# MILVLG/mmnas

Measured on AMD Instinct MI355X. Metric: supernet fwd+bwd steps/sec (VQA arch, bs=64), higher is better.
Workload: dtype f32 (bf16x6 split-operand MFMA, fp32 accumulate); 1 GPU; Net_Search supernet WEIGHT step: sample + fwd + BCE(sum) + bwd (+ gradient all-reduce), HSIZE 256, B=64/GPU, 100x2048 regions + 14 tokens, dropout 0.1 (search_vqa.py:279-292; BASELINE configs[2]); global_batch=64, parallelism=dp1, grad_allreduce=none, rccl_ranks=1, rank_id_sum_ok=True, lstm_fallback=False, dp_rows=1, dp_buckets=3, optimizer_in_step=False, gemm_split=6, hip_force_dev_kernarg=1

## Files before the change

include/mmnas_hip.h:

```cpp
#ifndef MMNAS_HIP_H
#define MMNAS_HIP_H

#include <stddef.h>
#include <stdint.h>

#ifdef __cplusplus
extern "C" {
#endif

#define MMNAS_ABI_VERSION 1

enum {
  MMNAS_OK = 0,
  MMNAS_E_SHAPE = -1,
  MMNAS_E_ARG = -2,
  MMNAS_E_LAUNCH = -3
};

enum {
  MMNAS_F_NORM = 1,
  MMNAS_F_RESIDUAL = 2,
  MMNAS_F_MASK = 4,
  MMNAS_F_REL = 8,
  MMNAS_F_SELF = 16,
  MMNAS_F_TRAIN = 32,
  MMNAS_F_RELRAW = 64
};

int mmnas_abi_version(void);
const char* mmnas_last_error(void);

int mmnas_dropout_mask(float* out, size_t n, float p, uint64_t seed, uint32_t site, void* stream);

enum { MMNAS_GEMM_NT = 0, MMNAS_GEMM_NN = 1, MMNAS_GEMM_TN = 2 };

typedef struct mmnas_gemm_group {
  int M;
  const float* A[3];
  const float* B[3];
  float* C;
  const float* bias;
  const float* residual;
  const float* gate;
  float* colsum;
  uint64_t drop_seed;
} mmnas_gemm_group;

#define MMNAS_GEMM_MAX_GROUPS 9

typedef struct mmnas_gemm_desc {
  int layout, ngroups, nseg;
  int N, K;
  int lda, ldb, ldc, ldres, ldgate;
  int relu, split_k;
  int accumulate;
  int b_planes;
  float alpha, gate_scale;
  float drop_p;
  uint32_t drop_site;
  uint64_t drop_seed;
  mmnas_gemm_group g[MMNAS_GEMM_MAX_GROUPS];
} mmnas_gemm_desc;

int mmnas_gemm(const mmnas_gemm_desc* d, void* stream);

int mmnas_gemm_ln(const mmnas_gemm_desc* d, const float* ln_a, const float* ln_b, float* y, float eps, void* stream);
int mmnas_set_gemm_ln(int on);

int mmnas_split_planes(const float* w, void* planes, size_t n, void* stream);

int mmnas_gemm_pair(const mmnas_gemm_desc* dgrad, const mmnas_gemm_desc* wgrad, void* stream);

int mmnas_lstm_supported(int E, int H);
int mmnas_lstm_fwd(const float* x_tm, const float* Wih, const float* Whh, const float* bias, float* xp, float* Hall,
                   float* Call, float* Gall, float* out, int T, int B, int E, int H, void* stream);
int mmnas_lstm_bwd(const float* dout, const float* Whh, const float* Call, const float* Gall, float* DG, float* dc,
                   float* scratch, int T, int B, int H, void* stream);

int mmnas_lstm_seq_supported(int H, int B);
int mmnas_lstm_seq_fwd(const float* xp, const float* bhh, const float* Whh, float* Hprev, float* Cs, float* Gall,
                       float* out, int T, int B, int H, void* stream);
int mmnas_lstm_seq_bwd(const float* dout, const float* Whh, const float* Cs, const float* Gall, float* DG, int T,
                       int B, int H, void* stream);
int mmnas_lstm_seq_timed_out(void* stream);

int mmnas_gemm_reload_tuning(void);

int mmnas_layernorm_fwd(const float* x, const float* a, const float* b, float* y,
                        int M, int d, float eps, void* stream);
int mmnas_layernorm_bwd(const float* x, const float* a, const float* dy, float* dx,
                        float* da, float* db, float* ddrop, float* dcol, float* ws,
                        float drop_p, uint64_t seed, uint32_t site,
                        int M, int d, float eps, void* stream);

size_t mmnas_layernorm_bwd_ws_floats(int M, int d);

int mmnas_colsum(const float* x, float* out, int M, int N, int ldx, void* stream);

int mmnas_eltwise_fwd(int kind, const float* x, float* y, size_t n, void* stream);
int mmnas_eltwise_bwd(int kind, const float* x, const float* dy, float* dx, size_t n, void* stream);
int mmnas_drop_add(const float* x, const float* res, float* y, size_t n, float drop_p, uint64_t seed,
                   uint32_t site, void* stream);
int mmnas_glu_fwd(const float* h, float* y, int M, int C, int relu, float drop_p, uint64_t seed,
                  uint32_t site, void* stream);
int mmnas_glu_bwd(const float* h, const float* dy, float* dh, int M, int C, int relu, float drop_p,
                  uint64_t seed, uint32_t site, void* stream);

int mmnas_row_is_zero(const float* f, uint8_t* mask, long rows, int d, void* stream);
int mmnas_glimpse1_supported(int K);
size_t mmnas_glimpse1_bwd_ws_floats(long rows, int K);
int mmnas_glimpse1_fwd(const float* x, const float* w, const float* b, float* y, long rows, int K, void* stream);
int mmnas_glimpse1_bwd(const float* dy, const float* x, const float* w, float* dx, float* dw, float* db, float* ws, long rows, int K,
                       void* stream);
int mmnas_attflat_pool_fwd(const float* logits, const float* x, const uint8_t* mask, float* probs, float* pooled,
                           int B, int S, int d, int G, void* stream);
int mmnas_attflat_pool_bwd(const float* probs, const float* x, const uint8_t* mask, const float* dpooled,
                           float* dlogits, float* dx, int B, int S, int d, int G, void* stream);

int mmnas_relation_embedding(const float* bbox, const int* nobj, float* out, int B, int S, void* stream);

int mmnas_semantic_embedding(const long* ques_ix, const int* nwords, const float* emb, float* out, int B, int S,
                             int E, long V, void* stream);

int mmnas_onehot_rows(float* out, int rows, int width, const int* idx_host, void* stream);

#define MMNAS_MIXED_MAX 8
size_t mmnas_mixed_sum_ws_floats(void);
int mmnas_node_mix_fwd(const float* const* z, const float* const* ln_a, const float* const* ln_b, int n, const float* gate,
                       float* out, int M, int d, float eps, void* stream);
int mmnas_node_mix_bwd(const float* const* z, const float* const* ln_a, const float* const* ln_b, int n, const float* gate,
                       const float* dout, float* d_active, int active, float* dgate, float* ws, int M, int d, float eps,
                       void* stream);
int mmnas_mixed_sum_fwd(const float* const* outs_host, int n, const float* gate, float* out, size_t count,
                        void* stream);
int mmnas_mixed_sum_bwd(const float* const* outs_host, int n, const float* gate, const float* dout,
                        float* d_active, int active, float* dgate, float* ws, size_t count, void* stream);
int mmnas_alpha_full_step(float* prob, const float* gate_grad, float* m, float* v, float* prob_grad, int rows,
                          int width, float lr, float beta1, float beta2, float eps, int step, void* stream);

int mmnas_embedding_bwd(const long* idx, const float* dy, float* dW, long n_tok, int E, long V, void* stream);
size_t mmnas_embedding_bwd_det_ws_floats(long n_tok, int E);
int mmnas_embedding_bwd_det(const long* idx, const float* dy, float* dW, float* ws, long n_tok, int E, long V, float scale,
                            void* stream);

int mmnas_rel_bias_fwd(const float* rel, const float* Wr, const float* br, float* biasT,
                       int B, int Sq, int Sk, int R, int H, void* stream);
int mmnas_rel_bias_bwd(const float* rel, const float* Wr, const float* br, const float* dbiasT,
                       float* drel, float* dWr, float* dbr, int accumulate_drel,
                       int B, int Sq, int Sk, int R, int H, void* stream);

int mmnas_rel_fused_supported(int C, int R, int H);
int mmnas_rel_fused_fwd(const float* raw, const float* Wy, const float* by, const float* Wr,
                        const float* br, float* biasT, int B, int Sq, int Sk, int C, int R, int H,
                        void* stream);
size_t mmnas_rel_fused_bwd_ws_floats(int B, int Sq, int Sk);
int mmnas_rel_fused_bwd(const float* raw, const float* Wy, const float* by, const float* Wr,
                        const float* br, const float* dbiasT, float* dWy, float* dby, float* dWr,
                        float* dbr, float* ws, int B, int Sq, int Sk, int C, int R, int H,
                        void* stream);
int mmnas_rel_fused_fwd_ragged(const float* raw, const float* Wy, const float* by, const float* Wr, const float* br,
                               float* biasT, int B, int S, int C, int R, int H, const int* off, void* stream);
int mmnas_rel_fused_bwd_ragged(const float* raw, const float* Wy, const float* by, const float* Wr, const float* br,
                               const float* dbiasT, float* dWy, float* dby, float* dWr, float* dbr, float* ws,
                               int B, int S, int C, int R, int H, const int* off, const int* tile_off, int ntiles, void* stream);

#define MMNAS_REL_MULTI_MAX 32
typedef struct mmnas_rel_multi {
  int B, S, C, R, H, n_ops;
  const float* raw;
  const float* Wy; const float* by;
  float* dWy; float* dby;
  const float* Wr[MMNAS_REL_MULTI_MAX];
  const float* br[MMNAS_REL_MULTI_MAX];
  float* biasT[MMNAS_REL_MULTI_MAX];
  const float* dbiasT[MMNAS_REL_MULTI_MAX];
  float* dWr[MMNAS_REL_MULTI_MAX]; float* dbr[MMNAS_REL_MULTI_MAX];
  const int* off; const int* tile_off; int ntiles, reserved;
  float* ws;
} mmnas_rel_multi;
int mmnas_rel_multi_supported(int C, int R, int H);
size_t mmnas_rel_multi_bwd_ws_floats(int B, int S);
int mmnas_rel_multi_fwd(const mmnas_rel_multi* m, void* stream);
int mmnas_rel_multi_bwd(const mmnas_rel_multi* m, void* stream);
int mmnas_set_rel_hoist(int on);
int mmnas_set_guided_hoist(int on);
int mmnas_set_rel_overlap(int on);

typedef struct mmnas_mha_desc {
  int B, H, Sq, Sk, dh;
  int ldq, ldk, ldv, ldo;
  const float* Q; const float* K; const float* V;
  const uint8_t* mask;
  const float* biasT;
  float* O;
  float* lse;
  float drop_p; uint32_t drop_site; uint64_t drop_seed;
  const float* dO;
  float* dQ; float* dK; float* dV;
  float* dbiasT;
  float* delta;
  const int* q_off; const int* k_off;
} mmnas_mha_desc;

int mmnas_mha_core_fwd(const mmnas_mha_desc* d, void* stream);
int mmnas_mha_core_bwd(const mmnas_mha_desc* d, void* stream);
int mmnas_mha_core_fwd_indexed(const mmnas_mha_desc* d, const int* kv_idx, void* stream);

typedef struct mmnas_att_op {
  int B, Sq, Sk, d, di, H, dh, R;
  int flags;
  float drop_p, eps;
  uint64_t seed;
  const float* xq;
  const float* xkv;
  const uint8_t* mask;
  const float* rel;
  const float* Wq; const float* Wk; const float* Wv;
  const float* Wm;
  const float* Wr; const float* br;
  const float* ln_a; const float* ln_b;
  float* y;
  void* save;
  void* ws;
  const float* dy;
  float* dxq;
  float* dxkv;
  float* drel;
  float* dWq; float* dWk; float* dWv; float* dWm;
  float* dWr; float* dbr; float* dln_a; float* dln_b;
  int C;
  const float* Wy; const float* by;
  float* dWy; float* dby;
  const int* q_off; const int* k_off;
  int Mq, Mk;
  const int* rel_tile_off;
  int rel_ntiles, reserved2;
} mmnas_att_op;

typedef struct mmnas_plan {
  size_t save_bytes, ws_fwd_bytes, ws_bwd_bytes;
} mmnas_plan;

int mmnas_set_small_ops(int on);
int mmnas_set_small_bwd(int on);
int mmnas_set_small_ffn(int on);
int mmnas_att_op_plan(const mmnas_att_op* op, mmnas_plan* plan);
int mmnas_att_op_fwd(const mmnas_att_op* op, void* stream);
int mmnas_att_op_bwd(const mmnas_att_op* op, void* stream);

typedef struct mmnas_mlp_op {
  int M, nl;
  int dims[4];
  int flags;
  float drop_p, eps;
  uint64_t seed;
  const float* x;
  const float* W[3];
  const float* b[3];
  const float* ln_a; const float* ln_b;
  float* y;
  void* save; void* ws;
  const float* dy;
  float* dx;
  float* dW[3]; float* db[3];
  float* dln_a; float* dln_b;
} mmnas_mlp_op;

int mmnas_mlp_op_plan(const mmnas_mlp_op* op, mmnas_plan* plan);
int mmnas_mlp_op_fwd(const mmnas_mlp_op* op, void* stream);
int mmnas_mlp_op_bwd(const mmnas_mlp_op* op, void* stream);

#define MMNAS_CHAIN_MAX_OPS 128
enum { MMNAS_CHAIN_ATT = 0, MMNAS_CHAIN_MLP = 1 };
typedef struct mmnas_chain_op {
  int kind, on_y;
  mmnas_att_op att;
  mmnas_mlp_op mlp;
  int node, cand, detached, reserved;
} mmnas_chain_op;
typedef struct mmnas_chain {
  int n_ops;
  const mmnas_chain_op* ops;
  int B, Sx, Sy, d;
  const float* x_in; const float* y_in;
  const uint8_t* x_mask; const uint8_t* y_mask;
  const float* x_rel; const float* y_rel;
  void* arena;
  float* x_out; float* y_out;
  const float* dx_out; const float* dy_out;
  float* dx_in; float* dy_in;
  int use_side_stream, reserved;
  void* const* marks;
  int mixed, gate_width;
  const float* gate;
  float* dgate;
  const int* y_off;
  const int* y_tile_off;
  int Ny, y_ntiles;
} mmnas_chain;
int mmnas_chain_plan(const mmnas_chain* c, size_t* arena_bytes);
int mmnas_chain_fwd(const mmnas_chain* c, void* stream);
int mmnas_chain_bwd(const mmnas_chain* c, void* stream);
int mmnas_chain_join(void* main_stream, void* waiting_stream);
int mmnas_set_chain_overlap(int on);

typedef struct mmnas_attflat_side {
  int S, reserved;
  const float* x; const uint8_t* mask;
  const float* W1; const float* b1; const float* W2; const float* b2; const float* Wm; const float* bm;
  float* dW1; float* db1; float* dW2; float* db2; float* dWm; float* dbm;
  uint64_t seed;
  float* dx;
  const int* off;
  int M, reserved2;
} mmnas_attflat_side;
typedef struct mmnas_head {
  int B, d, MID, G, OUT, ANS, flags, reserved;
  float drop_p, eps;
  mmnas_attflat_side sx, sy;
  const float* ln_a; const float* ln_b; float* dln_a; float* dln_b;
  const float* Wp; const float* bp; float* dWp; float* dbp;
  float* logits;
  const float* dlogits;
  void* arena;
} mmnas_head;
int mmnas_head_plan(const mmnas_head* hd, size_t* arena_bytes);
int mmnas_head_fwd(const mmnas_head* hd, void* stream);
// ... 64 lines not shown
```

mmnas_amd/_lib.py:

```python
import ctypes as C
import logging
import os

import torch

_HERE = os.path.dirname(os.path.abspath(__file__))
LIB_PATH = os.environ.get('MMNAS_LIB_PATH') or os.path.join(_HERE, 'lib', 'libmmnas_hip.so')

log = logging.getLogger('mmnas_amd')


def _launch_configuration():
    name = 'HIP_FORCE_DEV_KERNARG'
    if name in os.environ:
        return os.environ[name], 'inherited'
    if torch.cuda.is_initialized():
        log.warning('mmnas_amd was imported after HIP had initialised and %s is not set: kernel arguments go through host-visible '
                    'memory, the ~300 short launches of a step run 20-40 %% slower.  Export %s=1 or import mmnas / mmnas_amd '
                    'before the first CUDA call.', name, name)
        return None, 'unset_after_hip_init'
    os.environ[name] = '1'
    return '1', 'set_by_library'


# ... 44 lines not shown


class Plan(C.Structure):
    _fields_ = [('save_bytes', C.c_size_t), ('ws_fwd_bytes', C.c_size_t), ('ws_bwd_bytes', C.c_size_t)]


class MlpOp(C.Structure):
    _fields_ = [('M', C.c_int), ('nl', C.c_int), ('dims', C.c_int * 4), ('flags', C.c_int),
                ('drop_p', C.c_float), ('eps', C.c_float), ('seed', C.c_uint64),
                ('x', _fp), ('W', _fp * 3), ('b', _fp * 3), ('ln_a', _fp), ('ln_b', _fp), ('y', _fp),
                ('save', _fp), ('ws', _fp), ('dy', _fp), ('dx', _fp), ('dW', _fp * 3), ('db', _fp * 3),
                ('dln_a', _fp), ('dln_b', _fp)]


class ChainOp(C.Structure):
    _fields_ = [('kind', C.c_int), ('on_y', C.c_int), ('att', AttOp), ('mlp', MlpOp),
                ('node', C.c_int), ('cand', C.c_int), ('detached', C.c_int), ('reserved', C.c_int)]


class Chain(C.Structure):
    _fields_ = [('n_ops', C.c_int), ('ops', C.POINTER(ChainOp)), ('B', C.c_int), ('Sx', C.c_int), ('Sy', C.c_int),
                ('d', C.c_int), ('x_in', _fp), ('y_in', _fp), ('x_mask', _fp), ('y_mask', _fp), ('x_rel', _fp),
                ('y_rel', _fp), ('arena', _fp), ('x_out', _fp), ('y_out', _fp), ('dx_out', _fp), ('dy_out', _fp),
                ('dx_in', _fp), ('dy_in', _fp), ('use_side_stream', C.c_int), ('reserved', C.c_int),
                ('marks', C.c_void_p), ('mixed', C.c_int), ('gate_width', C.c_int), ('gate', _fp), ('dgate', _fp),
                ('y_off', _fp), ('y_tile_off', _fp), ('Ny', C.c_int), ('y_ntiles', C.c_int)]


CHAIN_MAX_OPS = 128


class AttFlatSide(C.Structure):
    _fields_ = [('S', C.c_int), ('reserved', C.c_int), ('x', _fp), ('mask', _fp), ('W1', _fp), ('b1', _fp), ('W2', _fp),
                ('b2', _fp), ('Wm', _fp), ('bm', _fp), ('dW1', _fp), ('db1', _fp), ('dW2', _fp), ('db2', _fp), ('dWm', _fp),
                ('dbm', _fp), ('seed', C.c_uint64), ('dx', _fp), ('off', _fp), ('M', C.c_int), ('reserved2', C.c_int)]


class Head(C.Structure):
    _fields_ = [('B', C.c_int), ('d', C.c_int), ('MID', C.c_int), ('G', C.c_int), ('OUT', C.c_int), ('ANS', C.c_int),
                ('flags', C.c_int), ('reserved', C.c_int), ('drop_p', C.c_float), ('eps', C.c_float),
                ('sx', AttFlatSide), ('sy', AttFlatSide), ('ln_a', _fp), ('ln_b', _fp), ('dln_a', _fp), ('dln_b', _fp),
                ('Wp', _fp), ('bp', _fp), ('dWp', _fp), ('dbp', _fp), ('logits', _fp), ('dlogits', _fp), ('arena', _fp)]


REL_MULTI_MAX = 32


class RelMulti(C.Structure):
    _fields_ = [('B', C.c_int), ('S', C.c_int), ('C', C.c_int), ('R', C.c_int), ('H', C.c_int), ('n_ops', C.c_int),
                ('raw', _fp), ('Wy', _fp), ('by', _fp), ('dWy', _fp), ('dby', _fp),
                ('Wr', _fp * REL_MULTI_MAX), ('br', _fp * REL_MULTI_MAX), ('biasT', _fp * REL_MULTI_MAX),
                ('dbiasT', _fp * REL_MULTI_MAX), ('dWr', _fp * REL_MULTI_MAX), ('dbr', _fp * REL_MULTI_MAX),
                ('off', _fp), ('tile_off', _fp), ('ntiles', C.c_int), ('reserved', C.c_int), ('ws', _fp)]


class ProfStat(C.Structure):
    _fields_ = [('ms', C.c_double), ('flops', C.c_double), ('bytes', C.c_double), ('launches', C.c_long)]


K_NAMES = ['gemm', 'mha_fwd', 'mha_bwd', 'rel_fwd', 'rel_bwd', 'rowops', 'lstm', 'small_ops']


class Segment(C.Structure):
    _fields_ = [('ptr', _fp), ('offset', C.c_uint64), ('n', C.c_uint64)]


_i, _f, _u32, _u64, _sz = C.c_int, C.c_float, C.c_uint32, C.c_uint64, C.c_size_t
SYMBOLS = {
    'mmnas_abi_version': (_i, []),
    'mmnas_last_error': (C.c_char_p, []),
    'mmnas_dropout_mask': (_i, [_fp, _sz, _f, _u64, _u32, _fp]),
    'mmnas_gemm': (_i, [C.POINTER(GemmDesc), _fp]),
    'mmnas_split_planes': (_i, [_fp, _fp, _sz, _fp]),
    'mmnas_gemm_ln': (_i, [C.POINTER(GemmDesc), _fp, _fp, _fp, _f, _fp]),
    'mmnas_set_gemm_ln': (_i, [_i]),
    'mmnas_gemm_pair': (_i, [C.POINTER(GemmDesc), C.POINTER(GemmDesc), _fp]),
    'mmnas_gemm_reload_tuning': (_i, []),
    'mmnas_lstm_supported': (_i, [_i, _i]),
    'mmnas_lstm_fwd': (_i, [_fp] * 9 + [_i, _i, _i, _i, _fp]),
    'mmnas_lstm_bwd': (_i, [_fp] * 7 + [_i, _i, _i, _fp]),
    'mmnas_lstm_seq_supported': (_i, [_i, _i]),
    'mmnas_set_small_ops': (_i, [_i]),
    'mmnas_set_small_bwd': (_i, [_i]),
    'mmnas_set_small_ffn': (_i, [_i]),
    'mmnas_set_chain_overlap': (_i, [_i]),
    'mmnas_lstm_seq_fwd': (_i, [_fp] * 7 + [_i, _i, _i, _fp]),
    'mmnas_lstm_seq_bwd': (_i, [_fp] * 5 + [_i, _i, _i, _fp]),
    'mmnas_lstm_seq_timed_out': (_i, [_fp]),
    'mmnas_layernorm_fwd': (_i, [_fp, _fp, _fp, _fp, _i, _i, _f, _fp]),
    'mmnas_layernorm_bwd': (_i, [_fp, _fp, _fp, _fp, _fp, _fp, _fp, _fp, _fp, _f, _u64, _u32, _i, _i, _f, _fp]),
    'mmnas_layernorm_bwd_ws_floats': (_sz, [_i, _i]),
    'mmnas_colsum': (_i, [_fp, _fp, _i, _i, _i, _fp]),
    'mmnas_eltwise_fwd': (_i, [_i, _fp, _fp, _sz, _fp]),
    'mmnas_eltwise_bwd': (_i, [_i, _fp, _fp, _fp, _sz, _fp]),
    'mmnas_drop_add': (_i, [_fp, _fp, _fp, _sz, _f, _u64, _u32, _fp]),
    'mmnas_glu_fwd': (_i, [_fp, _fp, _i, _i, _i, _f, _u64, _u32, _fp]),
    'mmnas_glu_bwd': (_i, [_fp, _fp, _fp, _i, _i, _i, _f, _u64, _u32, _fp]),
    'mmnas_rel_bias_fwd': (_i, [_fp, _fp, _fp, _fp, _i, _i, _i, _i, _i, _fp]),
    'mmnas_rel_bias_bwd': (_i, [_fp, _fp, _fp, _fp, _fp, _fp, _fp, _i, _i, _i, _i, _i, _i, _fp]),
    'mmnas_row_is_zero': (_i, [_fp, _fp, C.c_long, _i, _fp]),
    'mmnas_glimpse1_supported': (_i, [_i]),
    'mmnas_glimpse1_bwd_ws_floats': (_sz, [C.c_long, _i]),
    'mmnas_glimpse1_fwd': (_i, [_fp, _fp, _fp, _fp, C.c_long, _i, _fp]),
    'mmnas_glimpse1_bwd': (_i, [_fp, _fp, _fp, _fp, _fp, _fp, _fp, C.c_long, _i, _fp]),
    'mmnas_attflat_pool_fwd': (_i, [_fp, _fp, _fp, _fp, _fp, _i, _i, _i, _i, _fp]),
    'mmnas_attflat_pool_bwd': (_i, [_fp, _fp, _fp, _fp, _fp, _fp, _i, _i, _i, _i, _fp]),
    'mmnas_relation_embedding': (_i, [_fp, _fp, _fp, _i, _i, _fp]),
    'mmnas_semantic_embedding': (_i, [_fp, _fp, _fp, _fp, _i, _i, _i, C.c_long, _fp]),
    'mmnas_onehot_rows': (_i, [_fp, _i, _i, C.POINTER(C.c_int), _fp]),
    'mmnas_mixed_sum_ws_floats': (_sz, []),
    'mmnas_mixed_sum_fwd': (_i, [C.POINTER(_fp), _i, _fp, _fp, _sz, _fp]),
    'mmnas_mixed_sum_bwd': (_i, [C.POINTER(_fp), _i, _fp, _fp, _fp, _i, _fp, _fp, _sz, _fp]),
    'mmnas_alpha_full_step': (_i, [_fp, _fp, _fp, _fp, _fp, _i, _i, _f, _f, _f, _f, _i, _fp]),
    'mmnas_embedding_bwd': (_i, [_fp, _fp, _fp, C.c_long, _i, C.c_long, _fp]),
    'mmnas_node_mix_fwd': (_i, [_fp, _fp, _fp, _i, _fp, _fp, _i, _i, _f, _fp]),
    'mmnas_node_mix_bwd': (_i, [_fp, _fp, _fp, _i, _fp, _fp, _fp, _i, _fp, _fp, _i, _i, _f, _fp]),
    'mmnas_embedding_bwd_det': (_i, [_fp, _fp, _fp, _fp, C.c_long, _i, C.c_long, _f, _fp]),
    'mmnas_embedding_bwd_det_ws_floats': (_sz, [C.c_long, _i]),
    'mmnas_rel_fused_supported': (_i, [_i, _i, _i]),
    'mmnas_rel_fused_fwd': (_i, [_fp, _fp, _fp, _fp, _fp, _fp, _i, _i, _i, _i, _i, _i, _fp]),
    'mmnas_rel_fused_bwd_ws_floats': (_sz, [_i, _i, _i]),
    'mmnas_rel_fused_bwd': (_i, [_fp, _fp, _fp, _fp, _fp, _fp, _fp, _fp, _fp, _fp, _fp, _i, _i, _i, _i, _i, _i, _fp]),
    'mmnas_rel_fused_fwd_ragged': (_i, [_fp, _fp, _fp, _fp, _fp, _fp, _i, _i, _i, _i, _i, _fp, _fp]),
    'mmnas_rel_fused_bwd_ragged': (_i, [_fp] * 11 + [_i, _i, _i, _i, _i, _fp, _fp, _i, _fp]),
    'mmnas_rel_multi_supported': (_i, [_i, _i, _i]),
    'mmnas_rel_multi_bwd_ws_floats': (_sz, [_i, _i]),
    'mmnas_rel_multi_fwd': (_i, [C.POINTER(RelMulti), _fp]),
    'mmnas_rel_multi_bwd': (_i, [C.POINTER(RelMulti), _fp]),
    'mmnas_set_rel_hoist': (_i, [_i]),
    'mmnas_set_guided_hoist': (_i, [_i]),
    'mmnas_set_rel_overlap': (_i, [_i]),
    'mmnas_mha_core_fwd': (_i, [C.POINTER(MhaDesc), _fp]),
    'mmnas_mha_core_bwd': (_i, [C.POINTER(MhaDesc), _fp]),
    'mmnas_mha_core_fwd_indexed': (_i, [C.POINTER(MhaDesc), _fp, _fp]),
    'mmnas_itm_pair_head': (_i, [_fp] * 11 + [C.c_long, _i, _i, _f, _fp]),
    'mmnas_rank_matrix': (_i, [_fp, _i, _i, C.c_long, _fp, _fp, _fp, _fp, _fp, _fp]),
    'mmnas_row_topk': (_i, [_fp, _i, _i, C.c_long, _i, _fp, _fp, _fp]),
    'mmnas_vgd_targets': (_i, [_fp, _fp, _fp, _i, _i, C.c_double, _i, _fp, _fp, _fp, _fp, _fp, _fp, _fp]),
    'mmnas_vgd_ground': (_i, [_fp] * 5 + [_i, _i, C.c_double] + [_fp] * 7),
    'mmnas_vqa_answer': (_i, [_fp, _i, _i, C.c_long, _fp, C.c_long, _i, _i] + [_fp] * 4 + [_i] + [_fp] * 5),
    'mmnas_vqa_accuracy': (_i, [_fp] * 4 + [_i] * 4 + [_fp, _fp, _fp]),
    'mmnas_vqa_answer_targets': (_i, [_fp, _i, _i, _i, _fp, _fp, _fp]),
    'mmnas_vgd_loss_fwd': (_i, [_fp] * 6 + [_i] * 6 + [C.c_double, C.c_double] + [_fp] * 5),
    'mmnas_itm_triplet_loss_fwd': (_i, [_fp, _fp, _fp, C.c_long, _i, _f, _i, _fp, _fp, _fp]),
    'mmnas_loss_grad_scale': (_i, [_fp, _fp, _fp, _sz, _fp]),
    'mmnas_att_op_plan': (_i, [C.POINTER(AttOp), C.POINTER(Plan)]),
    'mmnas_att_op_fwd': (_i, [C.POINTER(AttOp), _fp]),
    'mmnas_att_op_bwd': (_i, [C.POINTER(AttOp), _fp]),
    'mmnas_mlp_op_plan': (_i, [C.POINTER(MlpOp), C.POINTER(Plan)]),
    'mmnas_mlp_op_fwd': (_i, [C.POINTER(MlpOp), _fp]),
    'mmnas_mlp_op_bwd': (_i, [C.POINTER(MlpOp), _fp]),
    'mmnas_chain_plan': (_i, [C.POINTER(Chain), C.POINTER(C.c_size_t)]),
    'mmnas_chain_fwd': (_i, [C.POINTER(Chain), _fp]),
    'mmnas_chain_bwd': (_i, [C.POINTER(Chain), _fp]),
    'mmnas_chain_join': (_i, [_fp, _fp]),
    'mmnas_head_plan': (_i, [C.POINTER(Head), C.POINTER(C.c_size_t)]),
    'mmnas_head_fwd': (_i, [C.POINTER(Head), _fp]),
    'mmnas_head_bwd': (_i, [C.POINTER(Head), _fp]),
    'mmnas_bce_logits_sum_fwd': (_i, [_fp, _fp, _fp, _sz, _fp]),
    'mmnas_bce_logits_bwd': (_i, [_fp, _fp, _fp, _fp, _sz, _fp]),
    'mmnas_im2col_seq': (_i, [_fp, _fp, _i, _i, _i, _i, _fp]),
    'mmnas_pack_rows': (_i, [_fp, _fp, _fp, _i, _i, _i, _fp]),
    'mmnas_unpack_rows': (_i, [_fp, _fp, _fp, _i, _i, _i, _fp]),
    'mmnas_pad_seq': (_i, [_fp, _fp, _i, _i, _i, _i, _i, C.c_long, _fp]),
    'mmnas_col2im_seq': (_i, [_fp, _fp, _i, _i, _i, _i, _fp]),
    'mmnas_dwconv_seq_fwd': (_i, [_fp, _fp, _fp, _fp, _i, _i, _i, _i, _fp]),
    'mmnas_dwconv_seq_bwd': (_i, [_fp, _fp, _fp, _fp, _fp, _fp, _i, _i, _i, _i, _fp]),
    'mmnas_pack_segments': (_i, [_fp, _i, _fp, _f, _i, _fp]),
    'mmnas_pack_segments_host': (_i, [C.POINTER(Segment), _i, _fp, _f, _i, _fp]),
    'mmnas_adam_step': (_i, [_fp, _fp, _fp, _fp, _sz, _f, _f, _f, _f, _f, _fp, _f, _i, _fp]),
    'mmnas_sumsq': (_i, [_fp, _sz, _fp, _fp]),
    'mmnas_prof_enable': (_i, [_i]),
    'mmnas_prof_collect': (_i, [C.POINTER(ProfStat)]),
}

# ... 50 lines not shown
```

mmnas_amd/csrc/common.h:

```cpp
#pragma once
#include <hip/hip_runtime.h>
#include <hip/hip_ext.h>
#include <stdint.h>
#include <stdio.h>
#include "../../include/mmnas_hip.h"
#include "rng.h"

namespace mmnas {

typedef float f32x4 __attribute__((ext_vector_type(4)));
typedef float f32x16 __attribute__((ext_vector_type(16)));

void set_error(const char* fmt, ...);
int check_launch(const char* what);

#define MMNAS_REQUIRE(cond, code, ...) \
  do { if (!(cond)) { ::mmnas::set_error(__VA_ARGS__); return (code); } } while (0)

template <int CTRL, int ROW_MASK>
__device__ __forceinline__ float dpp_move(float old, float src) {
  return __int_as_float(__builtin_amdgcn_update_dpp(__float_as_int(old), __float_as_int(src), CTRL, ROW_MASK, 0xf, false));
}
__device__ __forceinline__ float wave_sum(float v) {
  v += dpp_move<0xB1, 0xf>(0.f, v);
  v += dpp_move<0x4E, 0xf>(0.f, v);
  v += dpp_move<0x141, 0xf>(0.f, v);
  v += dpp_move<0x140, 0xf>(0.f, v);
  v += dpp_move<0x142, 0xa>(0.f, v);
  v += dpp_move<0x143, 0xc>(0.f, v);
  return __int_as_float(__builtin_amdgcn_readlane(__float_as_int(v), 63));
}
__device__ __forceinline__ float wave_max(float v) {
  constexpr float NI = -__builtin_inff();
  v = fmaxf(v, dpp_move<0xB1, 0xf>(NI, v));
  v = fmaxf(v, dpp_move<0x4E, 0xf>(NI, v));
  v = fmaxf(v, dpp_move<0x141, 0xf>(NI, v));
  v = fmaxf(v, dpp_move<0x140, 0xf>(NI, v));
  v = fmaxf(v, dpp_move<0x142, 0xa>(NI, v));
  v = fmaxf(v, dpp_move<0x143, 0xc>(NI, v));
  return __int_as_float(__builtin_amdgcn_readlane(__float_as_int(v), 63));
}

__device__ __forceinline__ int acc_row(int r, int hh) { return (r & 3) + 8 * (r >> 2) + 4 * hh; }

__device__ __forceinline__ f32x16 mfma32(float a, float b, f32x16 c) {
  return __builtin_amdgcn_mfma_f32_32x32x2f32(a, b, c, 0, 0, 0);
}

struct ProfScope {
  ProfScope(int kind, double flops, double bytes, hipStream_t st, const char* tag = nullptr);
  ~ProfScope();
  long idx_;
  hipStream_t st_;
};

struct ProfEvents { hipEvent_t start, stop; };
ProfEvents prof_launch_events();

#define MMNAS_LAUNCH(kernel, grid, block, shmem, stream, ...)                                            \
  do {                                                                                                   \
    const ::mmnas::ProfEvents pe_ = ::mmnas::prof_launch_events();                                       \
    if (pe_.stop) hipExtLaunchKernelGGL(kernel, grid, block, shmem, stream, pe_.start, pe_.stop, 0, __VA_ARGS__); \
    else hipLaunchKernelGGL(kernel, grid, block, shmem, stream, __VA_ARGS__);                            \
  } while (0)

bool prof_enabled();

struct AuxReduce {
  const float* part;
  int nrows, d;
  float* out[3];
};
int launch_aux_reduce(const AuxReduce& a, hipStream_t st);
int gemm_pair_aux(const mmnas_gemm_desc* dgrad, const mmnas_gemm_desc* wgrad, const AuxReduce* aux, hipStream_t st);
int gemm_wgrad_aux(const mmnas_gemm_desc* wgrad, const AuxReduce* aux, hipStream_t st);
int layernorm_bwd_deferred(const float* x, const float* a, const float* dy, float* dx, float* da, float* db, float* ddrop,
                           float* dcol, float* ws, float drop_p, uint64_t seed, uint32_t site, int M, int d, float eps,
                           hipStream_t st, AuxReduce* aux);


bool gemm_ln_applies(const mmnas_gemm_desc* d);
int gemm_ln(const mmnas_gemm_desc* d, const float* ln_a, const float* ln_b, float* y, int ldy, float eps, hipStream_t st);

bool glimpse1_supported(int MID);
int glimpse1_fwd(const float* h0, const float* w0, const float* b0, float* l0, long rows0, const float* h1, const float* w1,
                 const float* b1, float* l1, long rows1, int MID, hipStream_t st);
struct NodeLnBwd {
  float* dz; float* dt;
  float* part;
  DropCfg drop;
};
int node_mix_bwd_impl(const float* const* z, const float* const* ln_a, const float* const* ln_b, int n, const float* gate,
                      const float* dout, float* d_active, int active, float* dgate, float* ws, int M, int d, float eps,
                      hipStream_t stream, bool reduce, int* nwg_out, const NodeLnBwd* lnb = nullptr);
int mixed_reduce_many(const float* const* parts, float* const* dgates, const int* nwg, const int* n, int count, hipStream_t st);
int mha_core_fwd_pair(const mmnas_mha_desc* d0, const mmnas_mha_desc* d1, hipStream_t st);
int mha_core_fwd_indexed(const mmnas_mha_desc* d, const int* kv_idx, hipStream_t st);
int transpose2d(const float* in, float* out, int R, int C, hipStream_t st);
int glimpse1_bwd_blocks(long rows, int MID);
int glimpse1_bwd(const float* dlog, const float* h, const float* w2, float gate_scale, int gated, float* dh, float* db1, float* dW2,
                 float* part, long rows, int MID, hipStream_t st, AuxReduce* aux);

int attflat_pool_fwd_packed(const float* logits, const float* x, float* probs, float* pooled, int B, int S, int d, int G, const int* off, hipStream_t st);
int attflat_pool_bwd_packed(const float* probs, const float* x, const float* dpooled, float* dlogits, float* dx, int B, int S, int d, int G,
                            const int* off, hipStream_t st);

constexpr int ADD_MANY_MAX = 24;
int add_many(const float* const* srcs, int n, float* y, size_t count, hipStream_t st);

static inline int cdiv(long a, long b) { return (int)((a + b - 1) / b); }

}
```

mmnas_amd/csrc/gemm.hip:

```cpp
#include <stddef.h>
#include <string.h>
#include <map>
#include <mutex>
#include <utility>
#include <algorithm>
#include <climits>
#include "common.h"
#include "gemm_split.h"

namespace mmnas {

struct GemmGroupK {
  int M;
  int tile0;
  const float* A[3];
  const float* B[3];
  float* C;
  const float* bias;
  const float* residual;
  const float* gate;
  float* colsum;
  uint32_t seed_lo, site_key;
};

// ... 849 lines not shown
          float val = acc[i][j][r] * p.alpha + bv;
          if (has_relu) val = fmaxf(val, 0.f);
          if (has_drop) val *= drop_mult(gdrop, (uint32_t)row * (uint32_t)h.N + (uint32_t)col);
          if (has_gate) val = gatev[r] > 0.f ? val * p.gate_scale : 0.f;
          if (has_res) val += resv[r];
          if (has_acc) val += oldv[r];
          if (cok && row < Mg) { Cp[(size_t)row * p.ldc + col] = val; cs += val; }
        }
        if (csp != nullptr) {
          cs += __shfl_xor(cs, 32, 64);
          if (hh == 0 && cok) atomicAdd(csp + col, cs);
        }
      }
    }
#ifdef MMNAS_DBG_STAMP
    asm volatile("s_waitcnt vmcnt(0)" ::: "memory");
#endif
    MMNAS_LIFE(4);
  }
}

template <int BM, int BN, bool AKC, bool BKC, bool FAST, int NS, int EPI = 0, int PF = 1, bool BDMA = false, int LEAN = 0>
__global__ void __launch_bounds__(256, NS ? (BM == 128 ? (BN == 64 ? 2 : 1) : MMNAS_OCC_NS) : (BM == 128 ? MMNAS_OCC128 : MMNAS_OCC64)) gemm_kernel(const GemmK p) {
  __shared__ __attribute__((aligned(16))) float As[GemmShape<BM, BN, NS>::A_SZ], As1[GemmShape<BM, BN, NS>::A_SZ];
  __shared__ __attribute__((aligned(16))) float Bs[GemmShape<BM, BN, NS>::B_SZ], Bs1[GemmShape<BM, BN, NS>::B_SZ];
  __shared__ int s_old;
  gemm_body<BM, BN, AKC, BKC, FAST, NS, EPI, PF, BDMA, LEAN>(p, blockIdx.x, gridDim.x, 0, As, Bs, As1, Bs1, s_old);
}

struct AuxReduceK {
  const float* part;
  float* out[3];
  int nrows, d, ncb, njobs;
};

__device__ __forceinline__ void aux_reduce_body(const AuxReduceK& a, int job, float* red ) {
  const int w = job / a.ncb, cb = job - w * a.ncb;
  float* __restrict__ out = w == 0 ? a.out[0] : (w == 1 ? a.out[1] : a.out[2]);
  if (!out) return;
  const int cl = threadIdx.x & 15, g = threadIdx.x >> 4;
  const int c = cb * 16 + cl;
  float s0 = 0.f, s1 = 0.f, s2 = 0.f, s3 = 0.f;
  if (c < a.d) {
    const float* __restrict__ p = a.part + (size_t)w * a.d + c;
    const size_t rs = (size_t)3 * a.d;
    int b = g;
    for (; b + 48 < a.nrows; b += 64) {
      s0 += p[(size_t)b * rs];
      s1 += p[(size_t)(b + 16) * rs];
      s2 += p[(size_t)(b + 32) * rs];
      s3 += p[(size_t)(b + 48) * rs];
    }
    for (; b < a.nrows; b += 16) s0 += p[(size_t)b * rs];
  }
  red[g * 17 + cl] = (s0 + s1) + (s2 + s3);
  __syncthreads();
  if (g == 0 && c < a.d) {
    float t = 0.f;
#pragma unroll
    for (int i = 0; i < 16; ++i) t += red[i * 17 + cl];
    out[c] += t;
  }
}

template <int BM, int BN, int NS, int PF = 1, int LEAN0 = 0, int LEAN1 = 0>
__global__ void __launch_bounds__(256, NS ? MMNAS_OCC_NS : MMNAS_OCC64) gemm_pair_kernel(const GemmK q0, const GemmK q1, const int nwg0,
                                                                                    const int nwg0p, const AuxReduceK aux,
                                                                                    const int naux8) {
  __shared__ __attribute__((aligned(16))) float As[GemmShape<BM, BN, NS>::A_SZ], As1[GemmShape<BM, BN, NS>::A_SZ];
  __shared__ __attribute__((aligned(16))) float Bs[GemmShape<BM, BN, NS>::B_SZ], Bs1[GemmShape<BM, BN, NS>::B_SZ];
  __shared__ int s_old;
  int bid = blockIdx.x;
  if (bid < naux8) {
    if (bid < aux.njobs) aux_reduce_body(aux, bid, As);
    return;
  }
  bid -= naux8;
  if (bid < nwg0p) {
    if (bid < nwg0) gemm_body<BM, BN, true, false, true, NS, 0, PF, false, LEAN0>(q0, bid, nwg0, 0, As, Bs, As1, Bs1, s_old);
  } else {
    gemm_body<BM, BN, false, false, true, NS, 0, PF, false, LEAN1>(q1, bid - nwg0p, (int)gridDim.x - naux8 - nwg0p, (int)sizeof(GemmK), As, Bs, As1, Bs1, s_old);
  }
}

static int env_int(const char* name, int dflt) {
  const char* e = getenv(name);
  return e && e[0] ? atoi(e) : dflt;
}

struct Tuning { int tile, generic, sk, wgs, min_units, gm, xcd, split, pair, split_slots, split_p, pf, wide_min, split_minwg, hyb_t, lean, lean_maxb; bool loaded; };
static Tuning g_tune = {0, 0, 1, 0, 4, 0, 1, 3, 1, 0, 24, 2, 200, 256, 16, 3, 8 << 20, false};
static void load_tuning() {
  g_tune.tile = env_int("MMNAS_GEMM_TILE", 0);
  g_tune.generic = getenv("MMNAS_GEMM_GENERIC") != nullptr;
  g_tune.sk = env_int("MMNAS_GEMM_SK", 1);
  g_tune.wgs = env_int("MMNAS_GEMM_WGS", 0);
  g_tune.min_units = env_int("MMNAS_GEMM_MIN_UNITS", 4);
  if (g_tune.min_units < 1) g_tune.min_units = 1;
  g_tune.gm = env_int("MMNAS_GEMM_GM", 0);
  g_tune.xcd = env_int("MMNAS_GEMM_XCD", 1);
  const int sp = env_int("MMNAS_GEMM_SPLIT", 6);
  g_tune.split = sp == 3 ? 2 : (sp == 6 ? 3 : (sp == 1 ? 1 : 0));
  g_tune.pair = env_int("MMNAS_GEMM_PAIR", 1);
  g_tune.split_slots = env_int("MMNAS_GEMM_SPLIT_SLOTS", 0);
  g_tune.split_p = env_int("MMNAS_GEMM_SPLIT_P", 24);
  if (g_tune.split_p < 1) g_tune.split_p = 1;
  g_tune.split_minwg = env_int("MMNAS_GEMM_SPLIT_MINWG", 256);
  g_tune.pf = env_int("MMNAS_GEMM_PF", 2) == 1 ? 1 : 2;
  g_tune.hyb_t = env_int("MMNAS_GEMM_HYB_T", 16);
  g_tune.wide_min = env_int("MMNAS_GEMM_WIDE_MIN", 200);
  g_tune.lean = env_int("MMNAS_GEMM_LEAN", 3);
  g_tune.lean_maxb = env_int("MMNAS_GEMM_LEAN_MAXB", 8 << 20);
  g_tune.loaded = true;
}

constexpr int MAX_WGS = 1024;
constexpr size_t WS_SLOT_FLOATS = (size_t)2 * 512 * 128 * 128;
constexpr int MAX_CNT_TILES = 1 << 16;

struct SkWorkspace { float* ws; int* cnt; };
static std::mutex g_ws_mu;
static std::map<std::pair<int, hipStream_t>, SkWorkspace> g_ws;

static int get_workspace(hipStream_t st, SkWorkspace* out) {
  int dev = 0;
  if (hipGetDevice(&dev) != hipSuccess) { set_error("gemm: hipGetDevice failed"); return MMNAS_E_LAUNCH; }
  std::lock_guard<std::mutex> lk(g_ws_mu);
  auto key = std::make_pair(dev, st);
  auto it = g_ws.find(key);
  if (it == g_ws.end()) {
    SkWorkspace w{nullptr, nullptr};
    if (hipMalloc((void**)&w.ws, WS_SLOT_FLOATS * sizeof(float)) != hipSuccess ||
        hipMalloc((void**)&w.cnt, MAX_CNT_TILES * sizeof(int)) != hipSuccess ||
        hipMemset(w.cnt, 0, MAX_CNT_TILES * sizeof(int)) != hipSuccess) {
      set_error("gemm: cannot allocate the stream-K workspace (%zu MiB)", WS_SLOT_FLOATS * sizeof(float) >> 20);
      return MMNAS_E_LAUNCH;
    }
    it = g_ws.emplace(key, w).first;
  }
  *out = it->second;
  return MMNAS_OK;
}

int sk_workspace(hipStream_t st, float** ws, size_t* ws_floats, int** cnt, int* ncnt) {
  SkWorkspace w;
  const int rc = get_workspace(st, &w);
  if (rc) return rc;
  *ws = w.ws; *ws_floats = WS_SLOT_FLOATS; *cnt = w.cnt; *ncnt = MAX_CNT_TILES;
  return MMNAS_OK;
}

template <int BM, int BN, bool FAST, int NS, int PF = 1>
static int launch(GemmK& k, int layout, int nwg, hipStream_t st) {
  dim3 grid(nwg), block(256);
  switch (layout) {
    case MMNAS_GEMM_NT: MMNAS_LAUNCH((gemm_kernel<BM, BN, true, true, FAST, NS, 0, PF>), grid, block, 0, st, k); break;
    case MMNAS_GEMM_NN: MMNAS_LAUNCH((gemm_kernel<BM, BN, true, false, FAST, NS, 0, PF>), grid, block, 0, st, k); break;
    default: MMNAS_LAUNCH((gemm_kernel<BM, BN, false, false, FAST, NS, 0, PF>), grid, block, 0, st, k); break;
  }
  return check_launch("gemm");
}

}

using namespace mmnas;

// ... 243 lines not shown
  GemmPlan pl;
  const int rc = plan_gemm(d, (hipStream_t)stream, pl);
  if (rc) return rc;
  return launch_plan(pl, (hipStream_t)stream);
}

namespace mmnas {
int gemm_pair_aux(const mmnas_gemm_desc* dgrad, const mmnas_gemm_desc* wgrad, const AuxReduce* aux, hipStream_t st) {
  GemmPlan p0, p1;
  int rc;
  if ((rc = plan_gemm(dgrad, st, p0))) return rc;
  if ((rc = plan_gemm(wgrad, st, p1))) return rc;
  const bool pair = g_tune.pair && p0.fast && p1.fast && !p0.big && !p1.big && !p0.wide && !p1.wide && p0.layout == MMNAS_GEMM_NN &&
                    p1.layout == MMNAS_GEMM_TN && p1.k.mode != MODE_STREAM;
  if (!pair) {
    if (aux && (rc = launch_aux_reduce(*aux, st))) return rc;
    if ((rc = launch_plan(p0, st))) return rc;
    return launch_plan(p1, st);
  }
  AuxReduceK ak;
  memset(&ak, 0, sizeof(ak));
  if (aux && aux->part && g_tune.pair != 3) {
    ak.part = aux->part; ak.nrows = aux->nrows; ak.d = aux->d;
    for (int i = 0; i < 3; ++i) ak.out[i] = aux->out[i];
    ak.ncb = cdiv(aux->d, 16);
    ak.njobs = 3 * ak.ncb;
  } else if (aux && (rc = launch_aux_reduce(*aux, st))) return rc;
  const int naux8 = (ak.njobs + 7) / 8 * 8;
  char tag[96] = "";
  if (prof_enabled()) snprintf(tag, sizeof(tag), "PAIR %.44s | %.40s", p0.tag, p1.tag);
  ProfScope ps(MMNAS_K_GEMM, p0.flops + p1.flops, p0.bytes + p1.bytes, st, tag);
  const int nwg0p = (p0.nwg + 7) / 8 * 8;
  dim3 grid(naux8 + nwg0p + p1.nwg), block(256);
  switch (g_tune.split) {
    case 1: MMNAS_LAUNCH((gemm_pair_kernel<64, 64, 1, 2>), grid, block, 0, st, p0.k, p1.k, p0.nwg, nwg0p, ak, naux8); break;
    case 2: MMNAS_LAUNCH((gemm_pair_kernel<64, 64, 2>), grid, block, 0, st, p0.k, p1.k, p0.nwg, nwg0p, ak, naux8); break;
    case 3:
      if (p0.lean == 3 && p1.lean) MMNAS_LAUNCH((gemm_pair_kernel<64, 64, 3, 2, 3, 1>), grid, block, 0, st, p0.k, p1.k, p0.nwg, nwg0p, ak, naux8);
      else if (p0.lean == 3) MMNAS_LAUNCH((gemm_pair_kernel<64, 64, 3, 2, 3, 0>), grid, block, 0, st, p0.k, p1.k, p0.nwg, nwg0p, ak, naux8);
      else if (p0.lean == 1 && p1.lean) MMNAS_LAUNCH((gemm_pair_kernel<64, 64, 3, 2, 1, 1>), grid, block, 0, st, p0.k, p1.k, p0.nwg, nwg0p, ak, naux8);
      else if (p0.lean == 2 && p1.lean) MMNAS_LAUNCH((gemm_pair_kernel<64, 64, 3, 2, 2, 1>), grid, block, 0, st, p0.k, p1.k, p0.nwg, nwg0p, ak, naux8);
      else if (p0.lean) MMNAS_LAUNCH((gemm_pair_kernel<64, 64, 3, 2, 2, 0>), grid, block, 0, st, p0.k, p1.k, p0.nwg, nwg0p, ak, naux8);
      else if (p1.lean) MMNAS_LAUNCH((gemm_pair_kernel<64, 64, 3, 2, 0, 1>), grid, block, 0, st, p0.k, p1.k, p0.nwg, nwg0p, ak, naux8);
      else if (g_tune.pf == 2) MMNAS_LAUNCH((gemm_pair_kernel<64, 64, 3, 2>), grid, block, 0, st, p0.k, p1.k, p0.nwg, nwg0p, ak, naux8);
      else MMNAS_LAUNCH((gemm_pair_kernel<64, 64, 3>), grid, block, 0, st, p0.k, p1.k, p0.nwg, nwg0p, ak, naux8);
      break;
    default:
      if (g_tune.pf == 2) MMNAS_LAUNCH((gemm_pair_kernel<64, 64, 0, 2>), grid, block, 0, st, p0.k, p1.k, p0.nwg, nwg0p, ak, naux8);
      else MMNAS_LAUNCH((gemm_pair_kernel<64, 64, 0>), grid, block, 0, st, p0.k, p1.k, p0.nwg, nwg0p, ak, naux8);
      break;
  }
  return check_launch("gemm_pair");
}
}

namespace mmnas {
int gemm_wgrad_aux(const mmnas_gemm_desc* wgrad, const AuxReduce* aux, hipStream_t st) {
  GemmPlan p1;
  int rc;
  if ((rc = plan_gemm(wgrad, st, p1))) return rc;
  const bool ride = aux && aux->part && g_tune.pair && g_tune.pair != 3 && g_tune.split == 3 && g_tune.pf == 2 && p1.fast && !p1.big && !p1.wide &&
                    p1.layout == MMNAS_GEMM_TN && p1.k.mode != MODE_STREAM;
  if (!ride) {
    if (aux && (rc = launch_aux_reduce(*aux, st))) return rc;
    return launch_plan(p1, st);
  }
  AuxReduceK ak;
  memset(&ak, 0, sizeof(ak));
  ak.part = aux->part; ak.nrows = aux->nrows; ak.d = aux->d;
  for (int i = 0; i < 3; ++i) ak.out[i] = aux->out[i];
  ak.ncb = cdiv(aux->d, 16);
  ak.njobs = 3 * ak.ncb;
  const int naux8 = (ak.njobs + 7) / 8 * 8;
  char tag[96] = "";
  if (prof_enabled()) snprintf(tag, sizeof(tag), "WGRAD+AUX %.60s", p1.tag);
  ProfScope ps(MMNAS_K_GEMM, p1.flops, p1.bytes, st, tag);
  dim3 grid(naux8 + p1.nwg), block(256);
  if (p1.lean) MMNAS_LAUNCH((gemm_pair_kernel<64, 64, 3, 2, 0, 1>), grid, block, 0, st, p1.k, p1.k, 0, 0, ak, naux8);
  else MMNAS_LAUNCH((gemm_pair_kernel<64, 64, 3, 2>), grid, block, 0, st, p1.k, p1.k, 0, 0, ak, naux8);
  return check_launch("gemm_wgrad_aux");
}
}

extern "C" int mmnas_gemm_pair(const mmnas_gemm_desc* dgrad, const mmnas_gemm_desc* wgrad, void* stream) {
  return gemm_pair_aux(dgrad, wgrad, nullptr, (hipStream_t)stream);
}

namespace mmnas {
__global__ void __launch_bounds__(256) split_planes_kernel(const float4* __restrict__ w, uint2* __restrict__ p0, uint2* __restrict__ p1,
                                                           uint2* __restrict__ p2, size_t n4) {
  for (size_t i = (size_t)blockIdx.x * 256 + threadIdx.x; i < n4; i += (size_t)gridDim.x * 256) {
    const float4 v = w[i];
    unsigned a0, a1, a2, b0, b1, b2;
    split_pair<3>(v.x, v.y, a0, a1, a2);
    split_pair<3>(v.z, v.w, b0, b1, b2);
    p0[i] = make_uint2(a0, b0);
    p1[i] = make_uint2(a1, b1);
    p2[i] = make_uint2(a2, b2);
  }
}
}

extern "C" int mmnas_split_planes(const float* w, void* planes, size_t n, void* stream) {
  MMNAS_REQUIRE(w && planes, MMNAS_E_ARG, "split_planes: null pointer");
  MMNAS_REQUIRE(n > 0 && n % 8 == 0 && ((uintptr_t)w & 15) == 0 && ((uintptr_t)planes & 15) == 0, MMNAS_E_SHAPE,
                "split_planes: n = %zu must be a multiple of 8 and both buffers 16-byte aligned", n);
  const size_t n4 = n / 4;
  unsigned short* pl = (unsigned short*)planes;
  const int blocks = (int)std::min<size_t>((n4 + 255) / 256, 2048);
  MMNAS_LAUNCH(split_planes_kernel, dim3(blocks), dim3(256), 0, (hipStream_t)stream, (const float4*)w, (uint2*)pl, (uint2*)(pl + n),
               (uint2*)(pl + 2 * n), n4);
  return check_launch("split_planes");
}

namespace mmnas {
static int lstm_step_plan(GemmPlan& pl, const mmnas_gemm_desc& d, hipStream_t st, const char* who, int units_per_wg) {
  int rc = plan_gemm(&d, st, pl);
  if (rc) return rc;
  MMNAS_REQUIRE(pl.fast && !pl.big && !pl.wide, MMNAS_E_SHAPE, "%s: shape outside the step kernel's range (hidden size %% 32 == 0, aligned buffers)", who);
  GemmK& k = pl.k;
  k.n_full = k.full_per = k.sk_per = 0;
  if (units_per_wg <= 0 || units_per_wg >= k.T) {
    k.mode = MODE_TILE; k.P = k.T; pl.nwg = k.ntiles;
  } else {
    SkWorkspace w;
    if ((rc = get_workspace(st, &w))) return rc;
    k.ws = w.ws; k.cnt = w.cnt;
    k.mode = MODE_STREAM; k.P = units_per_wg; k.U = k.ntiles * k.T;
    pl.nwg = (k.U + k.P - 1) / k.P;
  }
  return MMNAS_OK;
}
}

extern "C" int mmnas_lstm_supported(int E, int H) { return E > 0 && H >= 32 && H % 32 == 0 && H <= 4096; }

extern "C" int mmnas_lstm_fwd(const float* x_tm, const float* Wih, const float* Whh, const float* bias, float* xp, float* Hall,
                              float* Call, float* Gall, float* out, int T, int B, int E, int H, void* stream) {
  MMNAS_REQUIRE(x_tm && Wih && Whh && bias && xp && Hall && Call && Gall && out, MMNAS_E_ARG, "lstm_fwd: null pointer");
  MMNAS_REQUIRE(T > 0 && B > 0 && mmnas_lstm_supported(E, H), MMNAS_E_SHAPE, "lstm_fwd: T=%d B=%d E=%d H=%d", T, B, E, H);
  hipStream_t st = (hipStream_t)stream;
  mmnas_gemm_desc d;
  memset(&d, 0, sizeof(d));
  d.layout = MMNAS_GEMM_NT; d.ngroups = 1; d.nseg = 1; d.N = 4 * H; d.K = E; d.lda = E; d.ldb = E; d.ldc = 4 * H;
  d.alpha = 1.f; d.gate_scale = 1.f; d.split_k = 1;
  d.g[0].M = T * B; d.g[0].A[0] = x_tm; d.g[0].B[0] = Wih; d.g[0].C = xp; d.g[0].bias = bias;
  int rc = mmnas_gemm(&d, stream);
  if (rc) return rc;
  const size_t bh = (size_t)B * H, bg = (size_t)B * 4 * H;
  for (int t = 0; t < T; ++t) {
    memset(&d, 0, sizeof(d));
    d.layout = MMNAS_GEMM_NT; d.ngroups = 1; d.nseg = 1; d.N = 4 * H; d.K = H; d.lda = H; d.ldb = H; d.ldc = H;
    d.ldres = 4 * H; d.alpha = 1.f; d.gate_scale = 1.f; d.split_k = 1;
    d.g[0].M = B; d.g[0].A[0] = Hall + t * bh; d.g[0].B[0] = Whh; d.g[0].C = Hall + (t + 1) * bh; d.g[0].residual = xp + t * bg;
    GemmPlan pl;
    if ((rc = lstm_step_plan(pl, d, st, "lstm_fwd", env_int("MMNAS_LSTM_FWD_P", 0)))) return rc;
    pl.k.lg_cprev = Call + t * bh; pl.k.lg_cout = Call + (t + 1) * bh; pl.k.lg_gates = Gall + t * bg;
    pl.k.lg_h2 = out + (size_t)t * H; pl.k.lg_ldh2 = T * H;
    ProfScope ps(MMNAS_K_GEMM, pl.flops, pl.bytes, st, pl.tag);
    MMNAS_LAUNCH((gemm_kernel<64, 64, true, true, true, 0, 1>), dim3(pl.nwg), dim3(256), 0, st, pl.k);
  }
  return check_launch("lstm_fwd");
}

extern "C" int mmnas_lstm_bwd(const float* dout, const float* Whh, const float* Call, const float* Gall, float* DG, float* dc,
                              float* scratch, int T, int B, int H, void* stream) {
// ... 32 lines not shown
```

mmnas_amd/csrc/ops.hip:

```cpp
#include <string.h>
#include <functional>
#include <vector>
#include "common.h"

namespace mmnas {

static inline size_t al(size_t n) { return (n + 255) & ~(size_t)255; }

struct Carver {
  char* base; size_t off;
  explicit Carver(void* p) : base((char*)p), off(0) {}
  float* take(size_t nfloats) { float* r = (float*)(base + off); off += al(nfloats * sizeof(float)); return r; }
};

static void gemm_init(mmnas_gemm_desc& g, int layout, int N, int K, int lda, int ldb, int ldc) {
  memset(&g, 0, sizeof(g));
  g.layout = layout; g.ngroups = 1; g.nseg = 1; g.N = N; g.K = K; g.lda = lda; g.ldb = ldb; g.ldc = ldc;
  g.alpha = 1.f; g.gate_scale = 1.f; g.split_k = 1;
}

struct AttLayout {
  size_t Mq, Mk;
  float *Q, *K, *V, *att, *stats, *z, *biasT;
  float *dz, *dt, *datt, *dQ, *dK, *dV, *delta, *dbiasT, *lnws, *relws;
// ... 121 lines not shown
      rc = op->q_off ? mmnas_rel_fused_fwd_ragged(op->rel, op->Wy, op->by, op->Wr, op->br, L.biasT, op->B, op->Sq, op->C, op->R,
                                                  op->H, op->q_off, stream)
                     : mmnas_rel_fused_fwd(op->rel, op->Wy, op->by, op->Wr, op->br, L.biasT, op->B, op->Sq, op->Sk, op->C, op->R,
                                           op->H, stream);
    } else {
      rc = mmnas_rel_bias_fwd(op->rel, op->Wr, op->br, L.biasT, op->B, op->Sq, op->Sk, op->R, op->H, stream);
    }
    if (rc) return rc;
  }
  if (desc_only) { att_core_desc(op, L, desc_only); return MMNAS_OK; }
  mmnas_mha_desc m;
  att_core_desc(op, L, &m);
  return mmnas_mha_core_fwd(&m, stream);
}

static void att_merge_group(const mmnas_att_op* op, const AttLayout& L, mmnas_gemm_group* g) {
  const bool norm = op->flags & MMNAS_F_NORM;
  memset(g, 0, sizeof(*g));
  g->M = (int)L.Mq; g->A[0] = L.att; g->B[0] = op->Wm; g->C = norm ? L.z : op->y;
  if (op->flags & MMNAS_F_RESIDUAL) g->residual = op->xq;
  g->drop_seed = op->seed;
}

static int att_fwd_args(const mmnas_att_op* op) {
  int rc = att_check(op, "att_op_fwd");
  if (rc) return rc;
  MMNAS_REQUIRE(op->xq && op->xkv && op->Wq && op->Wk && op->Wv && op->Wm && op->y && op->save, MMNAS_E_ARG,
                "att_op_fwd: null pointer");
  const int fl = op->flags;
  if (fl & MMNAS_F_NORM) MMNAS_REQUIRE(op->ln_a && op->ln_b, MMNAS_E_ARG, "att_op_fwd: NORM without ln parameters");
  if (fl & MMNAS_F_REL) MMNAS_REQUIRE(op->rel && op->Wr && op->br, MMNAS_E_ARG, "att_op_fwd: REL without rel/Wr/br");
  if (fl & MMNAS_F_MASK) MMNAS_REQUIRE(op->mask, MMNAS_E_ARG, "att_op_fwd: MASK without mask");
  return MMNAS_OK;
}
}

static int mmnas::att_fwd_impl(const mmnas_att_op* op, void* stream, bool defer_ln, bool* ln_done, bool rel_ready, bool kv_ready) {
  *ln_done = true;
  int rc = att_fwd_args(op);
  if (rc) return rc;
  const int fl = op->flags;
  const bool norm = fl & MMNAS_F_NORM;
  const bool drop = (fl & MMNAS_F_TRAIN) && op->drop_p > 0.f;
  AttLayout L = att_layout(op);
  const int d = op->d, di = op->di;
  if (sa_small_applies(op)) return sa_small_fwd(op, L.Q, L.K, L.V, L.att, L.stats, L.z, (hipStream_t)stream);

  mmnas_gemm_desc g;
  gemm_init(g, MMNAS_GEMM_NT, di, d, d, d, di);
  g.ngroups = kv_ready ? 1 : 3;
  att_qkv_groups(op, L, g.g);
  if ((rc = mmnas_gemm(&g, stream))) return rc;
  if ((rc = att_core_fwd(op, L, stream, nullptr, rel_ready))) return rc;
  gemm_init(g, MMNAS_GEMM_NT, d, di, di, di, d);
  att_merge_group(op, L, &g.g[0]);
  if (fl & MMNAS_F_RESIDUAL) g.ldres = d;
  if (drop) { g.drop_p = op->drop_p; g.drop_site = 1; g.drop_seed = op->seed; }
  if (norm && !defer_ln && gemm_ln_applies(&g)) return gemm_ln(&g, op->ln_a, op->ln_b, op->y, d, op->eps, (hipStream_t)stream);
  if ((rc = mmnas_gemm(&g, stream))) return rc;

  if (norm && defer_ln) { *ln_done = false; return MMNAS_OK; }
  if (norm) return mmnas_layernorm_fwd(L.z, op->ln_a, op->ln_b, op->y, (int)L.Mq, d, op->eps, stream);
  return MMNAS_OK;
}

namespace mmnas {
struct SideQueue {
  std::vector<std::function<int(hipStream_t)>> work;
  bool rel_only = false;
  int flush(hipStream_t main, hipStream_t side, hipEvent_t ev) {
    if (work.empty()) return MMNAS_OK;
    hipStream_t s = side;
    if (hipEventRecord(ev, main) != hipSuccess || hipStreamWaitEvent(side, ev, 0) != hipSuccess)
      s = main;
    for (auto& f : work) {
      const int rc = f(s);
      if (rc) return rc;
    }
    work.clear();
    return MMNAS_OK;
  }
};

static int att_bwd_impl(const mmnas_att_op* op, hipStream_t stream, SideQueue* sq, bool acc_kv = false, bool rel_defer = false, bool kv_defer = false,
                        const AuxReduce* ln_pre = nullptr) {
  const bool side = sq != nullptr && !sq->rel_only;
  const bool side_rel = sq != nullptr;
  int rc = att_check(op, "att_op_bwd");
  if (rc) return rc;
  MMNAS_REQUIRE(op->xq && op->xkv && op->Wq && op->Wk && op->Wv && op->Wm && op->save && op->ws && op->dy &&
                    op->dxq && op->dWq && op->dWk && op->dWv && op->dWm,
                MMNAS_E_ARG, "att_op_bwd: null pointer");
  const int fl = op->flags;
  const bool norm = fl & MMNAS_F_NORM, rel = fl & MMNAS_F_REL, self = fl & MMNAS_F_SELF;
  const bool drop = (fl & MMNAS_F_TRAIN) && op->drop_p > 0.f;
  if (!self) MMNAS_REQUIRE(op->dxkv, MMNAS_E_ARG, "att_op_bwd: dxkv required unless SELF");
  if (norm) MMNAS_REQUIRE(op->ln_a && op->dln_a && op->dln_b, MMNAS_E_ARG, "att_op_bwd: NORM gradients missing");
  if (rel) MMNAS_REQUIRE(op->rel && op->Wr && op->br && op->dWr && op->dbr, MMNAS_E_ARG, "att_op_bwd: REL gradients missing");
  AttLayout L = att_layout(op);
  const int d = op->d, di = op->di, Mq = (int)L.Mq, Mk = (int)L.Mk;

  if (!ln_pre && !sq && self && !rel && sa_small_bwd_applies(op)) {
    float* const dt_out = drop ? L.dt : (norm ? L.dz : nullptr);
    if ((rc = sa_small_bwd(op, L.Q, L.K, L.V, L.stats, L.z, dt_out, L.dQ, L.dK, L.dV, norm ? L.lnws : nullptr, stream))) return rc;
    mmnas_gemm_desc w4;
    gemm_init(w4, MMNAS_GEMM_TN, d, Mq, d, d, d);
    w4.ngroups = 4;
    w4.g[0].M = d; w4.g[0].A[0] = dt_out ? dt_out : op->dy; w4.g[0].B[0] = L.att; w4.g[0].C = op->dWm;
    w4.g[1].M = d; w4.g[1].A[0] = L.dQ; w4.g[1].B[0] = op->xq; w4.g[1].C = op->dWq;
    w4.g[2].M = d; w4.g[2].A[0] = L.dK; w4.g[2].B[0] = op->xq; w4.g[2].C = op->dWk;
    w4.g[3].M = d; w4.g[3].A[0] = L.dV; w4.g[3].B[0] = op->xq; w4.g[3].C = op->dWv;
    w4.accumulate = 1;
    AuxReduce red;
    red.part = norm ? L.lnws : nullptr; red.nrows = op->B; red.d = d;
    red.out[0] = op->dln_a; red.out[1] = op->dln_b; red.out[2] = nullptr;
    return gemm_wgrad_aux(&w4, &red, stream);
  }

  const float* dz = op->dy;
  const float* dt = op->dy;
  AuxReduce lnred;
  lnred.part = nullptr;
  if (norm && ln_pre) {
    lnred = *ln_pre;
    dz = L.dz; dt = drop ? L.dt : L.dz;
  } else if (norm) {
    if ((rc = layernorm_bwd_deferred(L.z, op->ln_a, op->dy, L.dz, op->dln_a, op->dln_b, drop ? L.dt : nullptr, nullptr,
                                     L.lnws, drop ? op->drop_p : 0.f, op->seed, 1, Mq, d, op->eps, (hipStream_t)stream, &lnred)))
      return rc;
    dz = L.dz; dt = drop ? L.dt : L.dz;
  } else if (drop) {
    if ((rc = mmnas_drop_add(op->dy, nullptr, L.dt, (size_t)Mq * d, op->drop_p, op->seed, 1, stream))) return rc;
    dt = L.dt;
  }

  mmnas_gemm_desc g, w, wm, w2;
  gemm_init(g, MMNAS_GEMM_NN, di, d, d, di, di);
  g.g[0].M = Mq; g.g[0].A[0] = dt; g.g[0].B[0] = op->Wm; g.g[0].C = L.datt;
  gemm_init(wm, MMNAS_GEMM_TN, di, Mq, d, di, di);
  wm.g[0].M = d; wm.g[0].A[0] = dt; wm.g[0].B[0] = L.att; wm.g[0].C = op->dWm;
  wm.accumulate = 1;
  if (side) { if ((rc = mmnas_gemm(&g, stream))) return rc; }
  else if ((rc = gemm_pair_aux(&g, &wm, &lnred, (hipStream_t)stream))) return rc;

  mmnas_mha_desc m;
  memset(&m, 0, sizeof(m));
  m.B = op->B; m.H = op->H; m.Sq = op->Sq; m.Sk = op->Sk; m.dh = op->dh;
  m.ldq = m.ldk = m.ldv = m.ldo = di;
  m.Q = L.Q; m.K = L.K; m.V = L.V; m.mask = (fl & MMNAS_F_MASK) ? op->mask : nullptr; m.biasT = L.biasT;
  m.O = L.att; m.lse = L.stats;
  m.drop_p = drop ? op->drop_p : 0.f; m.drop_site = 0; m.drop_seed = op->seed;
  m.dO = L.datt; m.dQ = L.dQ; m.dK = L.dK; m.dV = L.dV; m.dbiasT = L.dbiasT; m.delta = L.delta;
  m.q_off = op->q_off; m.k_off = op->k_off;
  if ((rc = mmnas_mha_core_bwd(&m, stream))) return rc;

  if (self) {
    gemm_init(w, MMNAS_GEMM_TN, d, Mq, di, d, d);
    w.ngroups = 3;
    w.g[0].M = di; w.g[0].A[0] = L.dQ; w.g[0].B[0] = op->xq;  w.g[0].C = op->dWq;
    w.g[1].M = di; w.g[1].A[0] = L.dK; w.g[1].B[0] = op->xkv; w.g[1].C = op->dWk;
    w.g[2].M = di; w.g[2].A[0] = L.dV; w.g[2].B[0] = op->xkv; w.g[2].C = op->dWv;
    w.accumulate = 1;
    gemm_init(g, MMNAS_GEMM_NN, d, di, di, d, d);
    g.nseg = 3;
    g.g[0].M = Mq; g.g[0].C = op->dxq;
    g.g[0].A[0] = L.dQ; g.g[0].B[0] = op->Wq;
    g.g[0].A[1] = L.dK; g.g[0].B[1] = op->Wk;
    g.g[0].A[2] = L.dV; g.g[0].B[2] = op->Wv;
    if (fl & MMNAS_F_RESIDUAL) { g.g[0].residual = dz; g.ldres = d; }
    if (side) {
      if ((rc = mmnas_gemm(&g, stream))) return rc;
    } else if ((rc = mmnas_gemm_pair(&g, &w, stream))) return rc;
  } else {
    gemm_init(w, MMNAS_GEMM_TN, d, Mq, di, d, d);
    w.g[0].M = di; w.g[0].A[0] = L.dQ; w.g[0].B[0] = op->xq; w.g[0].C = op->dWq;
    w.accumulate = 1;
    gemm_init(g, MMNAS_GEMM_NN, d, di, di, d, d);
    g.g[0].M = Mq; g.g[0].C = op->dxq; g.g[0].A[0] = L.dQ; g.g[0].B[0] = op->Wq;
    if (fl & MMNAS_F_RESIDUAL) { g.g[0].residual = dz; g.ldres = d; }
    if (side) {
      if ((rc = mmnas_gemm(&g, stream))) return rc;
    } else if ((rc = mmnas_gemm_pair(&g, &w, stream))) return rc;
    if (kv_defer) goto params;
    gemm_init(w2, MMNAS_GEMM_TN, d, Mk, di, d, d);
    w2.ngroups = 2;
    w2.g[0].M = di; w2.g[0].A[0] = L.dK; w2.g[0].B[0] = op->xkv; w2.g[0].C = op->dWk;
    w2.g[1].M = di; w2.g[1].A[0] = L.dV; w2.g[1].B[0] = op->xkv; w2.g[1].C = op->dWv;
    w2.accumulate = 1;
    gemm_init(g, MMNAS_GEMM_NN, d, di, di, d, d);
    g.nseg = 2;
    g.g[0].M = Mk; g.g[0].C = op->dxkv;
    g.g[0].A[0] = L.dK; g.g[0].B[0] = op->Wk;
    g.g[0].A[1] = L.dV; g.g[0].B[1] = op->Wv;
    if (acc_kv) g.accumulate = 1;
    if (side) {
      if ((rc = mmnas_gemm(&g, stream))) return rc;
    } else if ((rc = mmnas_gemm_pair(&g, &w2, stream))) return rc;
  }

params:
  if (side) {
    sq->work.push_back([lnred](hipStream_t s) { return launch_aux_reduce(lnred, s); });
    sq->work.push_back([wm](hipStream_t s) { return mmnas_gemm(&wm, s); });
    sq->work.push_back([w](hipStream_t s) { return mmnas_gemm(&w, s); });
    if (!self) sq->work.push_back([w2](hipStream_t s) { return mmnas_gemm(&w2, s); });
  }
  if (rel && rel_defer) return MMNAS_OK;
  if (rel && (fl & MMNAS_F_RELRAW)) {
    MMNAS_REQUIRE(op->Wy && op->by && op->dWy && op->dby, MMNAS_E_ARG, "att_op_bwd: RELRAW gradients missing");
    const mmnas_att_op o = *op;
    float* const dbiasT = L.dbiasT;
    float* const relws = L.relws;
    auto relb = [o, dbiasT, relws](hipStream_t s) {
      if (o.q_off)
        return mmnas_rel_fused_bwd_ragged(o.rel, o.Wy, o.by, o.Wr, o.br, dbiasT, o.dWy, o.dby, o.dWr, o.dbr, relws, o.B, o.Sq,
                                          o.C, o.R, o.H, o.q_off, o.rel_tile_off, o.rel_ntiles, s);
      return mmnas_rel_fused_bwd(o.rel, o.Wy, o.by, o.Wr, o.br, dbiasT, o.dWy, o.dby, o.dWr, o.dbr, relws, o.B, o.Sq, o.Sk,
                                 o.C, o.R, o.H, s);
    };
    if (side_rel) { sq->work.push_back(relb); return MMNAS_OK; }
    return relb(stream);
  }
  if (rel)
    return mmnas_rel_bias_bwd(op->rel, op->Wr, op->br, L.dbiasT, op->drel, op->dWr, op->dbr, 0, op->B, op->Sq,
                              op->Sk, op->R, op->H, stream);
  return MMNAS_OK;
}
}

extern "C" int mmnas_att_op_bwd(const mmnas_att_op* op, void* stream) {
  return att_bwd_impl(op, (hipStream_t)stream, nullptr);
}

namespace mmnas {

struct MlpLayout {
  float* h[3];
  float* z;
  float *dz, *dt, *dp[3], *lnws;
  size_t save_bytes, ws_bwd_bytes;
};

static MlpLayout mlp_layout(const mmnas_mlp_op* op) {
  MlpLayout L;
  const bool norm = op->flags & MMNAS_F_NORM;
  const bool drop = (op->flags & MMNAS_F_TRAIN) && op->drop_p > 0.f;
  const size_t M = (size_t)op->M;
  Carver s(op->save);
  L.h[0] = nullptr;
  for (int i = 1; i < 3; ++i) L.h[i] = (i < op->nl) ? s.take(M * op->dims[i]) : nullptr;
  L.z = norm ? s.take(M * op->dims[0]) : nullptr;
  L.save_bytes = s.off;
  size_t maxh = 4;
  for (int i = 1; i < op->nl; ++i) if ((size_t)op->dims[i] > maxh) maxh = op->dims[i];
  Carver w(op->ws);
  L.dz = norm ? w.take(M * op->dims[0]) : nullptr;
  L.dt = drop ? w.take(M * op->dims[0]) : nullptr;
  L.dp[0] = w.take(M * maxh);
  L.dp[1] = op->nl > 2 ? w.take(M * maxh) : nullptr;
  L.dp[2] = nullptr;
  L.lnws = norm ? w.take(mmnas_layernorm_bwd_ws_floats(op->M, op->dims[0])) : nullptr;
  L.ws_bwd_bytes = w.off;
  return L;
}

static int mlp_check(const mmnas_mlp_op* op, const char* who) {
  MMNAS_REQUIRE(op, MMNAS_E_ARG, "%s: null descriptor", who);
  MMNAS_REQUIRE(op->nl >= 1 && op->nl <= 3 && op->M > 0, MMNAS_E_SHAPE, "%s: nl=%d M=%d", who, op->nl, op->M);
  MMNAS_REQUIRE(op->dims[0] == op->dims[op->nl], MMNAS_E_SHAPE, "%s: in/out width differ (%d vs %d)", who,
                op->dims[0], op->dims[op->nl]);
  for (int i = 0; i <= op->nl; ++i)
    MMNAS_REQUIRE(op->dims[i] > 0 && op->dims[i] % 4 == 0, MMNAS_E_SHAPE, "%s: dims[%d]=%d", who, i, op->dims[i]);
  return MMNAS_OK;
}

}

extern "C" int mmnas_mlp_op_plan(const mmnas_mlp_op* op, mmnas_plan* plan) {
  int rc = mlp_check(op, "mlp_op_plan");
  if (rc) return rc;
  MMNAS_REQUIRE(plan, MMNAS_E_ARG, "mlp_op_plan: null plan");
  mmnas_mlp_op tmp = *op;
  tmp.save = nullptr; tmp.ws = nullptr;
  MlpLayout L = mlp_layout(&tmp);
  plan->save_bytes = L.save_bytes ? L.save_bytes : 256;
  plan->ws_fwd_bytes = 256;
  plan->ws_bwd_bytes = L.ws_bwd_bytes;
  return MMNAS_OK;
}

namespace mmnas {
static int mlp_fwd_impl(const mmnas_mlp_op* op, void* stream, bool defer_ln, bool* ln_done);
}
extern "C" int mmnas_mlp_op_fwd(const mmnas_mlp_op* op, void* stream) {
  bool done;
  return mmnas::mlp_fwd_impl(op, stream, false, &done);
}
static int mmnas::mlp_fwd_impl(const mmnas_mlp_op* op, void* stream, bool defer_ln, bool* ln_done) {
  *ln_done = true;
  int rc = mlp_check(op, "mlp_op_fwd");
  if (rc) return rc;
  MMNAS_REQUIRE(op->x && op->y && op->save, MMNAS_E_ARG, "mlp_op_fwd: null pointer");
  const int fl = op->flags;
  const bool norm = fl & MMNAS_F_NORM;
  const bool drop = (fl & MMNAS_F_TRAIN) && op->drop_p > 0.f;
  if (norm) MMNAS_REQUIRE(op->ln_a && op->ln_b, MMNAS_E_ARG, "mlp_op_fwd: NORM without ln parameters");
  MlpLayout L = mlp_layout(op);
  const int d = op->dims[0];
  if (!(norm && defer_ln) && ffn_small_applies(op)) return ffn_small_fwd(op, L.h[1], L.z, (hipStream_t)stream);
  const float* in = op->x;
  mmnas_gemm_desc g;
  for (int i = 0; i < op->nl; ++i) {
    MMNAS_REQUIRE(op->W[i], MMNAS_E_ARG, "mlp_op_fwd: W[%d] null", i);
    const bool last = i == op->nl - 1;
    gemm_init(g, MMNAS_GEMM_NT, op->dims[i + 1], op->dims[i], op->dims[i], op->dims[i], op->dims[i + 1]);
    g.g[0].M = op->M; g.g[0].A[0] = in; g.g[0].B[0] = op->W[i]; g.g[0].bias = op->b[i];
    if (drop) { g.drop_p = op->drop_p; g.drop_seed = op->seed; g.drop_site = last ? 1u : (i == 0 ? 0u : 2u); }
    if (last) {
      g.g[0].C = norm ? L.z : op->y;
      if (fl & MMNAS_F_RESIDUAL) { g.g[0].residual = op->x; g.ldres = d; }
    } else {
      g.relu = 1;
      g.g[0].C = L.h[i + 1];
    }
    if (last && norm && !defer_ln && gemm_ln_applies(&g)) return gemm_ln(&g, op->ln_a, op->ln_b, op->y, d, op->eps, (hipStream_t)stream);
    if ((rc = mmnas_gemm(&g, stream))) return rc;
    in = L.h[i + 1];
  }
  if (norm && defer_ln) { *ln_done = false; return MMNAS_OK; }
  if (norm) return mmnas_layernorm_fwd(L.z, op->ln_a, op->ln_b, op->y, op->M, d, op->eps, stream);
  return MMNAS_OK;
}

namespace mmnas {
static int mlp_bwd_impl(const mmnas_mlp_op* op, hipStream_t stream, SideQueue* sq, const AuxReduce* ln_pre = nullptr) {
  const bool side = sq != nullptr && !sq->rel_only;
  int rc = mlp_check(op, "mlp_op_bwd");
  if (rc) return rc;
  MMNAS_REQUIRE(op->x && op->save && op->ws && op->dy && op->dx, MMNAS_E_ARG, "mlp_op_bwd: null pointer");
  const int fl = op->flags;
  const bool norm = fl & MMNAS_F_NORM;
  const bool drop = (fl & MMNAS_F_TRAIN) && op->drop_p > 0.f;
  MlpLayout L = mlp_layout(op);
  const int d = op->dims[0], M = op->M, nl = op->nl;
  for (int i = 0; i < nl; ++i)
    MMNAS_REQUIRE(op->W[i] && op->dW[i], MMNAS_E_ARG, "mlp_op_bwd: W/dW[%d] null", i);

  const float* dz = op->dy;
  const float* dt = op->dy;
  bool last_bias_done = false;
  AuxReduce lnred;
  lnred.part = nullptr;
  if (norm) {
    MMNAS_REQUIRE(op->ln_a && op->dln_a && op->dln_b, MMNAS_E_ARG, "mlp_op_bwd: NORM gradients missing");
    float* dcol = (drop && op->db[nl - 1]) ? op->db[nl - 1] : nullptr;
    if (ln_pre) lnred = *ln_pre;
    else if ((rc = layernorm_bwd_deferred(L.z, op->ln_a, op->dy, L.dz, op->dln_a, op->dln_b, drop ? L.dt : nullptr, dcol,
                                          L.lnws, drop ? op->drop_p : 0.f, op->seed, 1, M, d, op->eps, (hipStream_t)stream, &lnred)))
      return rc;
    dz = L.dz; dt = drop ? L.dt : L.dz;
    last_bias_done = dcol != nullptr;
  } else if (drop) {
    if ((rc = mmnas_drop_add(op->dy, nullptr, L.dt, (size_t)M * d, op->drop_p, op->seed, 1, stream))) return rc;
    dt = L.dt;
  }

  const float gate_scale = drop ? 1.0f / (1.0f - op->drop_p) : 1.0f;
  const float* dpre = dt;
  mmnas_gemm_desc g;
  mmnas_gemm_desc wd[3];
  const bool last_colsum = op->db[nl - 1] && !last_bias_done;
  if (last_colsum && !side)
    if ((rc = mmnas_colsum(dpre, op->db[nl - 1], M, op->dims[nl], op->dims[nl], stream))) return rc;
  for (int i = nl - 1; i >= 0; --i) {
    const float* hin = i == 0 ? op->x : L.h[i];
    const int nout = op->dims[i + 1], nin = op->dims[i];
    mmnas_gemm_desc& w = wd[i];
    gemm_init(w, MMNAS_GEMM_TN, nin, M, nout, nin, nin);
    w.g[0].M = nout; w.g[0].A[0] = dpre; w.g[0].B[0] = hin; w.g[0].C = op->dW[i];
    w.accumulate = 1;
    gemm_init(g, MMNAS_GEMM_NN, nin, nout, nout, nin, nin);
    g.g[0].M = M; g.g[0].A[0] = dpre; g.g[0].B[0] = op->W[i];
    if (i == 0) {
      g.g[0].C = op->dx;
      if (fl & MMNAS_F_RESIDUAL) { g.g[0].residual = dz; g.ldres = d; }
    } else {
      float* out = L.dp[(nl - 1 - i) % 3];
      g.g[0].C = out;
      g.g[0].gate = L.h[i]; g.ldgate = nin; g.gate_scale = gate_scale;
      g.g[0].colsum = op->db[i - 1];
    }
    if (side) {
      if ((rc = mmnas_gemm(&g, stream))) return rc;
    } else if ((rc = gemm_pair_aux(&g, &w, i == nl - 1 ? &lnred : nullptr, (hipStream_t)stream))) return rc;
    if (i > 0) dpre = g.g[0].C;
  }
  if (side) {
    sq->work.push_back([lnred](hipStream_t s) { return launch_aux_reduce(lnred, s); });
    if (last_colsum) {
      float* const db = op->db[nl - 1];
      const int n = op->dims[nl];
      sq->work.push_back([dt, db, M, n](hipStream_t s) { return mmnas_colsum(dt, db, M, n, n, s); });
    }
    for (int i = nl - 1; i >= 0; --i) {
      const mmnas_gemm_desc w = wd[i];
      sq->work.push_back([w](hipStream_t s) { return mmnas_gemm(&w, s); });
    }
  }
  return MMNAS_OK;
}
}

extern "C" int mmnas_mlp_op_bwd(const mmnas_mlp_op* op, void* stream) {
  return mlp_bwd_impl(op, (hipStream_t)stream, nullptr);
}

#include <map>
#include <mutex>
#include <utility>
namespace mmnas {

struct ChainLayout {
  size_t y[MMNAS_CHAIN_MAX_OPS], save[MMNAS_CHAIN_MAX_OPS], ws[MMNAS_CHAIN_MAX_OPS], dx[MMNAS_CHAIN_MAX_OPS],
      tmp[MMNAS_CHAIN_MAX_OPS];
  size_t dpre, encdy, relws, total;
  int last_x, last_y, first_x, first_y, n_guided;
  size_t nout[MMNAS_CHAIN_MAX_OPS], ndact[MMNAS_CHAIN_MAX_OPS], mixws;
};

static int chain_check(const mmnas_chain* c, const char* who) {
  MMNAS_REQUIRE(c && c->ops, MMNAS_E_ARG, "%s: null chain", who);
  MMNAS_REQUIRE(c->n_ops >= 1 && c->n_ops <= MMNAS_CHAIN_MAX_OPS, MMNAS_E_SHAPE, "%s: %d operators (1..%d)", who, c->n_ops, MMNAS_CHAIN_MAX_OPS);
  MMNAS_REQUIRE(c->B > 0 && c->Sx > 0 && c->Sy > 0 && c->d > 0, MMNAS_E_SHAPE, "%s: B=%d Sx=%d Sy=%d d=%d", who, c->B, c->Sx, c->Sy, c->d);
  if (c->y_off) MMNAS_REQUIRE(c->Ny > 0 && c->Ny <= c->B * c->Sy && c->Sy <= 128 && !c->use_side_stream, MMNAS_E_ARG,
                              "%s: ragged decoder stream: Ny=%d of B*Sy=%d rows, Sy=%d <= 128, single stream", who, c->Ny, c->B * c->Sy, c->Sy);
  bool seen_y = false;
  for (int i = 0; i < c->n_ops; ++i) {
    const mmnas_chain_op& o = c->ops[i];
    MMNAS_REQUIRE(o.kind == MMNAS_CHAIN_ATT || o.kind == MMNAS_CHAIN_MLP, MMNAS_E_ARG, "%s: operator %d: kind %d", who, i, o.kind);
    if (o.on_y) seen_y = true;
    else MMNAS_REQUIRE(!seen_y, MMNAS_E_ARG, "%s: encoder operators must precede the decoder's (operator %d)", who, i);
    if (o.kind == MMNAS_CHAIN_ATT && !(o.att.flags & MMNAS_F_SELF))
      MMNAS_REQUIRE(o.on_y, MMNAS_E_ARG, "%s: operator %d: guided attention needs the decoder stream", who, i);
  }
  if (c->mixed) {
    MMNAS_REQUIRE(c->gate && c->gate_width >= 1 && c->gate_width <= MMNAS_MIXED_MAX, MMNAS_E_ARG, "%s: mixed chain without a gate block (width %d)", who, c->gate_width);
    MMNAS_REQUIRE(!c->use_side_stream, MMNAS_E_ARG, "%s: mixed chains run on one stream", who);
    MMNAS_REQUIRE(c->d <= 1024, MMNAS_E_SHAPE, "%s: mixed chains need d <= 1024", who);
    int node = -1, live = 0, count = 0;
    for (int i = 0; i < c->n_ops; ++i) {
      const mmnas_chain_op& o = c->ops[i];
      if (o.node != node) {
        MMNAS_REQUIRE(o.node == node + 1, MMNAS_E_ARG, "%s: operator %d: node %d after node %d", who, i, o.node, node);
        MMNAS_REQUIRE(node < 0 || live == 1, MMNAS_E_ARG, "%s: node %d has %d differentiated candidates (exactly one)", who, node, live);
        node = o.node; live = 0; count = 0;
      } else {
        MMNAS_REQUIRE(o.on_y == c->ops[i - 1].on_y, MMNAS_E_ARG, "%s: node %d mixes the two streams", who, node);
      }
      MMNAS_REQUIRE(o.cand >= 0 && o.cand < c->gate_width, MMNAS_E_ARG, "%s: operator %d: candidate %d outside the gate row", who, i, o.cand);
      MMNAS_REQUIRE(++count <= MMNAS_MIXED_MAX, MMNAS_E_SHAPE, "%s: node %d has more than %d candidates", who, node, MMNAS_MIXED_MAX);
      live += o.detached ? 0 : 1;
    }
    MMNAS_REQUIRE(live == 1, MMNAS_E_ARG, "%s: node %d has %d differentiated candidates (exactly one)", who, node, live);
  }
  return MMNAS_OK;
}

static inline size_t chain_rows_y(const mmnas_chain* c) { return c->y_off ? (size_t)c->Ny : (size_t)c->B * c->Sy; }

static void chain_op_setup(const mmnas_chain* c, int i, mmnas_att_op& a, mmnas_mlp_op& m) {
  const mmnas_chain_op& o = c->ops[i];
  const int S = o.on_y ? c->Sy : c->Sx;
  if (o.kind == MMNAS_CHAIN_ATT) {
    a = o.att;
    a.B = c->B; a.d = c->d; a.Sq = S;
    const bool self = a.flags & MMNAS_F_SELF;
    a.Sk = self ? S : c->Sx;
// ... 411 lines not shown
      }
      gemm_init(g, MMNAS_GEMM_NT, c->d, f.di, f.di, f.di, c->d);
      g.ngroups = ng;
      for (int j = 0; j < ng; ++j) att_merge_group(&ga[j], gl[j], &g.g[j]);
      if (f.flags & MMNAS_F_RESIDUAL) g.ldres = c->d;
      if (drop) { g.drop_p = f.drop_p; g.drop_site = 1; g.drop_seed = f.seed; }
      if ((rc = mmnas_gemm(&g, st))) return rc;
    }
    for (int i = i0; i < i1; ++i) {
      const mmnas_chain_op& o = c->ops[i];
      mmnas_att_op a; mmnas_mlp_op m;
      chain_op_setup(c, i, a, m);
      bool ln_done = true;
      bool staged = false;
      for (int j = 0; j < ng; ++j) staged |= gidx[j] == i;
      if (staged) {
        ln_done = !(a.flags & MMNAS_F_NORM);
        if (a.flags & MMNAS_F_NORM) eps = a.eps;
        chain_cand_view(c, L, i, ln_done, &z[i - i0], &la[i - i0], &lb[i - i0]);
        continue;
      }
      if (o.kind == MMNAS_CHAIN_ATT) {
        a.xq = cur;
        a.xkv = (a.flags & MMNAS_F_SELF) ? cur : cur_x;
        a.y = (float*)(base + L.y[i]); a.save = base + L.save[i]; a.ws = base + L.ws[i];
        if ((rc = att_fwd_impl(&a, st, true, &ln_done, RG.hoisted[i]))) return rc;
        if (a.flags & MMNAS_F_NORM) eps = a.eps;
      } else {
        m.x = cur; m.y = (float*)(base + L.y[i]); m.save = base + L.save[i]; m.ws = base + L.ws[i];
        if ((rc = mlp_fwd_impl(&m, st, true, &ln_done))) return rc;
        if (m.flags & MMNAS_F_NORM) eps = m.eps;
      }
      chain_cand_view(c, L, i, ln_done, &z[i - i0], &la[i - i0], &lb[i - i0]);
    }
    const float* zs[MMNAS_MIXED_MAX] = {nullptr}; const float* as[MMNAS_MIXED_MAX] = {nullptr}; const float* bs[MMNAS_MIXED_MAX] = {nullptr};
    int width = 0;
    for (int i = i0; i < i1; ++i) {
      const int k = c->ops[i].cand;
      zs[k] = z[i - i0]; as[k] = la[i - i0]; bs[k] = lb[i - i0];
      if (k + 1 > width) width = k + 1;
    }
    float* out = i0 == L.last_x ? c->x_out : (i0 == L.last_y ? c->y_out : (float*)(base + L.nout[i0]));
    const int M = oy ? (int)chain_rows_y(c) : c->B * c->Sx;
    if ((rc = mmnas_node_mix_fwd(zs, as, bs, width, c->gate + (size_t)c->ops[i0].node * c->gate_width, out, M, c->d, eps, st))) return rc;
    if (oy) cur_y = out; else cur_x = out;
    i0 = i1;
  }
  if (L.last_x < 0 && hipMemcpyAsync(c->x_out, c->x_in, nx, hipMemcpyDeviceToDevice, st) != hipSuccess) return MMNAS_E_LAUNCH;
  if (L.last_y < 0 && hipMemcpyAsync(c->y_out, c->y_in, ny, hipMemcpyDeviceToDevice, st) != hipSuccess) return MMNAS_E_LAUNCH;
  return MMNAS_OK;
}

static int chain_bwd_mixed(const mmnas_chain* c, hipStream_t st, const ChainLayout& L) {
  MMNAS_REQUIRE(c->dgate, MMNAS_E_ARG, "chain_bwd: mixed chain without a gate-gradient block");
  char* base = (char*)c->arena;
  const size_t ex = (size_t)c->B * c->Sx * c->d, ey = chain_rows_y(c) * c->d;
  float* dpre = (float*)(base + L.dpre);
  int rc;
  GuidedSet GS;
  chain_guided_set(c, true, true, GS);
  int Gm = -1;
  for (int i = 0; i < c->n_ops && Gm < 0; ++i)
    if (GS.hoisted[i]) Gm = i;
  const float* enc_grad = nullptr;
  if (L.n_guided > GS.n && hipMemsetAsync(dpre, 0, ex * sizeof(float), st) != hipSuccess) return MMNAS_E_LAUNCH;
  int starts[MMNAS_CHAIN_MAX_OPS + 1], nn = 0;
  for (int i = 0; i < c->n_ops; ++i)
    if (i == 0 || c->ops[i].node != c->ops[i - 1].node) starts[nn++] = i;
  starts[nn] = c->n_ops;
  auto node_out = [&](int i0) -> const float* { return i0 == L.last_x ? c->x_out : (i0 == L.last_y ? c->y_out : (const float*)(base + L.nout[i0])); };
  auto input_of = [&](int k) -> const float* {
    const bool oy = c->ops[starts[k]].on_y;
    for (int j = k - 1; j >= 0; --j)
      if ((bool)c->ops[starts[j]].on_y == oy) return node_out(starts[j]);
    return oy ? c->y_in : c->x_in;
  };
  const float* x_final = L.last_x >= 0 ? c->x_out : c->x_in;
  const float* cur_dy = c->dy_out;
  const float* red_part[MMNAS_CHAIN_MAX_OPS]; float* red_out[MMNAS_CHAIN_MAX_OPS]; int red_nwg[MMNAS_CHAIN_MAX_OPS], red_n[MMNAS_CHAIN_MAX_OPS];
  int n_red = 0;
  RelGroups RG;
  chain_rel_groups(c, L, true, RG);
  SideCtx* rel_bwd_side = nullptr;
  for (int k = nn - 1; k >= 0; --k) {
    const int i0 = starts[k], i1 = starts[k + 1];
    const bool oy = c->ops[i0].on_y;
    if (!oy && i0 == L.last_x) {
      MMNAS_REQUIRE(c->dx_out || L.n_guided, MMNAS_E_ARG, "chain_bwd: no gradient reaches the encoder (dx_out NULL, no guided operator)");
      if (enc_grad) cur_dy = enc_grad;
      else if (c->dx_out && L.n_guided) {
        float* g0 = (float*)(base + L.encdy);
        if ((rc = mmnas_drop_add(c->dx_out, dpre, g0, ex, 0.f, 0, 0, st))) return rc;
        cur_dy = g0;
      } else cur_dy = c->dx_out ? c->dx_out : dpre;
    }
    const float* zs[MMNAS_MIXED_MAX] = {nullptr}; const float* as[MMNAS_MIXED_MAX] = {nullptr}; const float* bs[MMNAS_MIXED_MAX] = {nullptr};
    int width = 0, act = -1, act_op = -1;
    float eps = 1e-6f;
    for (int i = i0; i < i1; ++i) {
      const int kc = c->ops[i].cand;
      chain_cand_view(c, L, i, chain_ln_done_in_op(c, i), &zs[kc], &as[kc], &bs[kc]);
      if (kc + 1 > width) width = kc + 1;
      if (!c->ops[i].detached) { act = kc; act_op = i; }
      const mmnas_chain_op& o = c->ops[i];
      if (o.kind == MMNAS_CHAIN_ATT) { if (o.att.flags & MMNAS_F_NORM) eps = o.att.eps; }
      else if (o.mlp.flags & MMNAS_F_NORM) eps = o.mlp.eps;
    }
    const float* nin = input_of(k);
    float* dact = (float*)(base + L.ndact[i0]);
    const int M = oy ? (int)chain_rows_y(c) : c->B * c->Sx;
    const size_t grow = (size_t)c->ops[i0].node * c->gate_width;
    const mmnas_chain_op& o = c->ops[act_op];
    mmnas_att_op a; mmnas_mlp_op m;
    chain_op_setup(c, act_op, a, m);
    float* dx = i0 == L.first_x ? c->dx_in : (i0 == L.first_y ? c->dy_in : (float*)(base + L.dx[act_op]));
    NodeLnBwd lnb;
    lnb.dz = nullptr;
    AuxReduce lnpre;
    lnpre.part = nullptr;
    if (o.kind == MMNAS_CHAIN_ATT) {
      const bool self = a.flags & MMNAS_F_SELF;
      a.xq = nin;
      a.xkv = self ? nin : x_final;
      a.save = base + L.save[act_op]; a.ws = base + L.ws[act_op];
      a.dy = dact; a.dxq = dx;
      a.dxkv = self ? nullptr : dpre;
      a.drel = nullptr;
      if (node_lnb_on() && (a.flags & MMNAS_F_NORM) && c->d <= 256 && !(self && !(a.flags & MMNAS_F_REL) && sa_small_bwd_applies(&a))) {
        const AttLayout AL = att_layout(&a);
        const bool drop = (a.flags & MMNAS_F_TRAIN) && a.drop_p > 0.f;
        lnb.dz = AL.dz; lnb.dt = drop ? AL.dt : nullptr; lnb.part = AL.lnws;
        lnb.drop = make_drop(drop ? a.drop_p : 0.f, a.seed, 1);
        lnpre.part = AL.lnws; lnpre.d = c->d;
        lnpre.out[0] = a.dln_a; lnpre.out[1] = a.dln_b; lnpre.out[2] = nullptr;
      }
    } else {
      m.x = nin; m.save = base + L.save[act_op]; m.ws = base + L.ws[act_op];
      m.dy = dact; m.dx = dx;
      if (node_lnb_on() && (m.flags & MMNAS_F_NORM) && c->d <= 256) {
        const MlpLayout ML = mlp_layout(&m);
        const bool drop = (m.flags & MMNAS_F_TRAIN) && m.drop_p > 0.f;
        lnb.dz = ML.dz; lnb.dt = drop ? ML.dt : nullptr; lnb.part = ML.lnws;
        lnb.drop = make_drop(drop ? m.drop_p : 0.f, m.seed, 1);
        lnpre.part = ML.lnws; lnpre.d = c->d;
        lnpre.out[0] = m.dln_a; lnpre.out[1] = m.dln_b; lnpre.out[2] = (drop && m.db[m.nl - 1]) ? m.db[m.nl - 1] : nullptr;
      }
    }
    {
      float* wsk = (float*)(base + L.mixws) + (size_t)k * mmnas_mixed_sum_ws_floats();
      int nwg = 0;
      if ((rc = node_mix_bwd_impl(zs, as, bs, width, c->gate + grow, cur_dy, dact, act, c->dgate + grow, wsk, M, c->d, eps, st, false, &nwg,
                                  lnb.dz ? &lnb : nullptr)))
        return rc;
      if (nwg > 0) { red_part[n_red] = wsk; red_out[n_red] = c->dgate + grow; red_nwg[n_red] = nwg; red_n[n_red] = width; ++n_red; }
      lnpre.nrows = nwg;
    }
    if (o.kind == MMNAS_CHAIN_ATT) {
      const bool self = a.flags & MMNAS_F_SELF;
      if ((rc = att_bwd_impl(&a, st, nullptr, !self, RG.hoisted[act_op], GS.hoisted[act_op], lnb.dz ? &lnpre : nullptr))) return rc;
      if (GS.n && act_op == Gm) {
        float* g0 = (float*)(base + L.encdy);
        if ((rc = chain_guided_kv_bwd(c, L, GS, x_final, c->dx_out, GS.n < L.n_guided ? dpre : nullptr, g0, st))) return rc;
        enc_grad = g0;
      }
    } else {
      if ((rc = mlp_bwd_impl(&m, st, nullptr, lnb.dz ? &lnpre : nullptr))) return rc;
    }
    cur_dy = dx;
    hipStream_t mark_stream = st;
    if (i0 == L.first_y && !RG.groups[1].empty()) {
      SideCtx* rsc = (rel_overlap_on() && L.last_x >= 0) ? side_ctx(st, true) : nullptr;
      if (rsc) {
        if ((rc = ev_fork(st, rsc->side, rsc->ovl[2]))) return rc;
        if ((rc = chain_rel_bwd(RG, 1, rsc->side))) return rc;
        rel_bwd_side = rsc;
        mark_stream = rsc->side;
      } else if ((rc = chain_rel_bwd(RG, 1, st))) return rc;
    }
    if (i0 == L.first_x && !RG.groups[0].empty()) {
      if (rel_bwd_side) { if ((rc = ev_fork(rel_bwd_side->side, st, rel_bwd_side->ovl[3]))) return rc; rel_bwd_side = nullptr; }
      if ((rc = chain_rel_bwd(RG, 0, st))) return rc;
    }
    if (c->marks && c->marks[act_op] && hipEventRecord((hipEvent_t)c->marks[act_op], mark_stream) != hipSuccess) {
      set_error("chain_bwd: cannot record the mark event of operator %d", act_op);
      return MMNAS_E_LAUNCH;
    }
  }
  if (rel_bwd_side && (rc = ev_fork(rel_bwd_side->side, st, rel_bwd_side->ovl[3]))) return rc;
  if (n_red && (rc = mixed_reduce_many(red_part, red_out, red_nwg, red_n, n_red, st))) return rc;
  if (L.first_y < 0 && hipMemcpyAsync(c->dy_in, c->dy_out, ey * sizeof(float), hipMemcpyDeviceToDevice, st) != hipSuccess) return MMNAS_E_LAUNCH;
  if (L.first_x < 0) {
    const float* g0 = c->dx_out;
    if (enc_grad) g0 = enc_grad;
    else if (c->dx_out && L.n_guided) {
      if ((rc = mmnas_drop_add(c->dx_out, dpre, c->dx_in, ex, 0.f, 0, 0, st))) return rc;
      g0 = nullptr;
    } else if (!c->dx_out) g0 = dpre;
    if (g0 && hipMemcpyAsync(c->dx_in, g0, ex * sizeof(float), hipMemcpyDeviceToDevice, st) != hipSuccess) return MMNAS_E_LAUNCH;
  }
  return MMNAS_OK;
}
}

extern "C" int mmnas_chain_fwd(const mmnas_chain* c, void* stream) {
  int rc = chain_check(c, "chain_fwd");
  if (rc) return rc;
  MMNAS_REQUIRE(c->x_in && c->y_in && c->x_out && c->y_out && c->arena, MMNAS_E_ARG, "chain_fwd: null pointer");
  hipStream_t st = (hipStream_t)stream;
  ChainLayout L;
  if ((rc = chain_layout(c, L))) return rc;
  if (c->mixed) return chain_fwd_mixed(c, st, L);
  char* base = (char*)c->arena;
  const float* cur_x = c->x_in;
  const float* cur_y = c->y_in;
  const size_t nx = (size_t)c->B * c->Sx * c->d * sizeof(float), ny = chain_rows_y(c) * c->d * sizeof(float);
  RelGroups RG;
  chain_rel_groups(c, L, false, RG);
  const int G = first_guided(c);
  const bool ovl = chain_overlap_on() && !c->use_side_stream && L.last_x >= 0 && L.first_y >= 0 && G > L.first_y;
  int rel_join_at = -1;
  SideCtx* rsc = nullptr;
  if (!ovl && rel_overlap_on() && !RG.groups[1].empty() && L.last_x >= 0 && (rsc = side_ctx(st, true)) != nullptr) {
    for (int i = L.first_y; i < c->n_ops && rel_join_at < 0; ++i)
      if (RG.hoisted[i] && c->ops[i].on_y) rel_join_at = i;
  }
  if (rel_join_at >= 0) {
    if ((rc = ev_fork(st, rsc->side, rsc->ovl[0]))) return rc;
    if ((rc = chain_rel_fwd(RG, rsc->side, 1))) return rc;
    if ((rc = chain_rel_fwd(RG, st, 0))) return rc;
  } else if ((rc = chain_rel_fwd(RG, st))) return rc;
  GuidedSet GS;
  chain_guided_set(c, false, !ovl, GS);
  auto run = [&](int i, hipStream_t s) -> int {
    const mmnas_chain_op& o = c->ops[i];
    mmnas_att_op a; mmnas_mlp_op m;
    chain_op_setup(c, i, a, m);
    const float* cur = o.on_y ? cur_y : cur_x;
    float* out = i == L.last_x ? c->x_out : (i == L.last_y ? c->y_out : (float*)(base + L.y[i]));
    int r;
    if (o.kind == MMNAS_CHAIN_ATT) {
      a.xq = cur;
      a.xkv = (a.flags & MMNAS_F_SELF) ? cur : cur_x;
      a.y = out; a.save = base + L.save[i]; a.ws = base + L.ws[i];
      bool done;
      if ((r = att_fwd_impl(&a, s, false, &done, RG.hoisted[i], GS.hoisted[i]))) return r;
    } else {
      m.x = cur; m.y = out; m.save = base + L.save[i]; m.ws = base + L.ws[i];
      if ((r = mmnas_mlp_op_fwd(&m, s))) return r;
    }
    if (o.on_y) cur_y = out; else cur_x = out;
    return MMNAS_OK;
  };
  if (!ovl) {
    for (int i = 0; i < c->n_ops; ++i) {
      if (GS.n && i == G && (rc = chain_guided_kv_fwd(c, L, GS, cur_x, st))) return rc;
      if (i == rel_join_at && (rc = ev_fork(rsc->side, st, rsc->ovl[1]))) return rc;
      if ((rc = run(i, st))) return rc;
    }
  } else {
    SideCtx* sc = side_ctx(st, true);
    MMNAS_REQUIRE(sc, MMNAS_E_LAUNCH, "chain_fwd: cannot create the encoder stream");
    if ((rc = ev_fork(st, sc->enc, sc->ovl[0]))) return rc;
    int ie = L.first_x, id = L.first_y;
    while (ie <= L.last_x || id < G) {
      if (ie <= L.last_x && (rc = run(ie++, sc->enc))) return rc;
      if (id < G && (rc = run(id++, st))) return rc;
    }
    if ((rc = ev_fork(sc->enc, st, sc->ovl[1]))) return rc;
    for (int i = G; i < c->n_ops; ++i)
      if ((rc = run(i, st))) return rc;
  }
  if (L.last_x < 0 && hipMemcpyAsync(c->x_out, c->x_in, nx, hipMemcpyDeviceToDevice, st) != hipSuccess) return MMNAS_E_LAUNCH;
  if (L.last_y < 0 && hipMemcpyAsync(c->y_out, c->y_in, ny, hipMemcpyDeviceToDevice, st) != hipSuccess) return MMNAS_E_LAUNCH;
  return MMNAS_OK;
}

extern "C" int mmnas_chain_bwd(const mmnas_chain* c, void* stream) {
  int rc = chain_check(c, "chain_bwd");
  if (rc) return rc;
  MMNAS_REQUIRE(c->x_in && c->y_in && c->x_out && c->y_out && c->arena && c->dy_out && c->dx_in && c->dy_in, MMNAS_E_ARG,
                "chain_bwd: null pointer");
  hipStream_t st = (hipStream_t)stream;
  ChainLayout L;
  if ((rc = chain_layout(c, L))) return rc;
  if (c->mixed) return chain_bwd_mixed(c, st, L);
  SideCtx* sc = c->use_side_stream ? side_ctx(st, true) : nullptr;
  MMNAS_REQUIRE(!c->use_side_stream || sc, MMNAS_E_LAUNCH, "chain_bwd: cannot create the side stream");
  hipStream_t side = sc ? sc->side : nullptr;
  if (sc) sc->used = true;
  SideQueue q;
  q.rel_only = c->use_side_stream == 2;
  SideQueue* sq = sc ? &q : nullptr;
  static const bool per_op = getenv("MMNAS_SIDE_FLUSH") && !strcmp(getenv("MMNAS_SIDE_FLUSH"), "op");
  char* base = (char*)c->arena;
  const size_t ex = (size_t)c->B * c->Sx * c->d, ey = chain_rows_y(c) * c->d;
  float* dpre = (float*)(base + L.dpre);
  auto input_of = [&](int i) -> const float* {
    const bool oy = c->ops[i].on_y;
    for (int j = i - 1; j >= 0; --j)
      if ((bool)c->ops[j].on_y == oy) return j == L.last_x ? c->x_out : (j == L.last_y ? c->y_out : (const float*)(base + L.y[j]));
    return oy ? c->y_in : c->x_in;
  };
  const float* x_final = L.last_x >= 0 ? c->x_out : c->x_in;
  const int G = first_guided(c);
  const bool ovl = chain_overlap_on() && !c->use_side_stream && L.last_x >= 0 && L.first_y >= 0 && G > L.first_y;
  RelGroups RG;
  if (!ovl) chain_rel_groups(c, L, true, RG);
  GuidedSet GS;
  chain_guided_set(c, true, !ovl, GS);
  const float* enc_grad = nullptr;
  SideCtx* rel_bwd_side = nullptr;
  if (L.n_guided > GS.n && hipMemsetAsync(dpre, 0, ex * sizeof(float), st) != hipSuccess) return MMNAS_E_LAUNCH;
  auto run = [&](int i, hipStream_t s, const float* dyi, const float** dxo) -> int {
    const mmnas_chain_op& o = c->ops[i];
    mmnas_att_op a; mmnas_mlp_op m;
    chain_op_setup(c, i, a, m);
    float* dx = i == L.first_x ? c->dx_in : (i == L.first_y ? c->dy_in : (float*)(base + L.dx[i]));
    int r;
    if (o.kind == MMNAS_CHAIN_ATT) {
      const bool self = a.flags & MMNAS_F_SELF;
      a.xq = input_of(i);
      a.xkv = self ? a.xq : x_final;
      a.save = base + L.save[i]; a.ws = base + L.ws[i];
      a.dy = dyi; a.dxq = dx;
      a.dxkv = self ? nullptr : dpre;
      a.drel = nullptr;
      if ((r = att_bwd_impl(&a, s, sq, !self, RG.hoisted[i], GS.hoisted[i]))) return r;
      if (GS.n && i == G) {
        float* g0 = (float*)(base + L.encdy);
        if ((r = chain_guided_kv_bwd(c, L, GS, x_final, c->dx_out, GS.n < L.n_guided ? dpre : nullptr, g0, s))) return r;
        enc_grad = g0;
      }
    } else {
      m.x = input_of(i); m.save = base + L.save[i]; m.ws = base + L.ws[i];
      m.dy = dyi; m.dx = dx;
      if ((r = mlp_bwd_impl(&m, s, sq))) return r;
    }
    *dxo = dx;
    hipStream_t mark_stream = s;
    if (i == L.first_y && !RG.groups[1].empty()) {
      SideCtx* rsc = (rel_overlap_on() && L.last_x >= 0 && !sq) ? side_ctx(st, true) : nullptr;
      if (rsc) {
        if ((r = ev_fork(s, rsc->side, rsc->ovl[2]))) return r;
        if ((r = chain_rel_bwd(RG, 1, rsc->side))) return r;
        rel_bwd_side = rsc;
        mark_stream = rsc->side;
      } else if ((r = chain_rel_bwd(RG, 1, s))) return r;
    }
    if (i == L.first_x && !RG.groups[0].empty()) {
      if (rel_bwd_side) { if ((r = ev_fork(rel_bwd_side->side, s, rel_bwd_side->ovl[3]))) return r; rel_bwd_side = nullptr; }
      if ((r = chain_rel_bwd(RG, 0, s))) return r;
    }
    if (!ovl && c->marks && c->marks[i] && hipEventRecord((hipEvent_t)c->marks[i], mark_stream) != hipSuccess) {
      set_error("chain_bwd: cannot record the mark event of operator %d", i);
      return MMNAS_E_LAUNCH;
    }
    return MMNAS_OK;
  };
  auto encoder_dy = [&](hipStream_t s, const float** out) -> int {
    MMNAS_REQUIRE(c->dx_out || L.n_guided, MMNAS_E_ARG, "chain_bwd: no gradient reaches the encoder (dx_out NULL, no guided operator)");
    if (enc_grad) { *out = enc_grad; return MMNAS_OK; }
    if (c->dx_out && L.n_guided) {
      float* g0 = (float*)(base + L.encdy);
      const int r = mmnas_drop_add(c->dx_out, dpre, g0, ex, 0.f, 0, 0, s);
      if (r) return r;
      *out = g0;
    } else *out = c->dx_out ? c->dx_out : dpre;
    return MMNAS_OK;
  };
  const float* cur_dy = c->dy_out;
  if (!ovl) {
    for (int i = c->n_ops - 1; i >= 0; --i) {
      if (sq && i == L.last_x && (rc = q.flush(st, side, sc->ev[0]))) return rc;
      if (!c->ops[i].on_y && i == L.last_x && (rc = encoder_dy(st, &cur_dy))) return rc;
      if ((rc = run(i, st, cur_dy, &cur_dy))) return rc;
      if (sq && per_op && (rc = q.flush(st, side, sc->ev[i + 1]))) return rc;
    }
    if (sq && (rc = q.flush(st, side, sc->ev[1]))) return rc;
  } else {
    SideCtx* oc = side_ctx(st, true);
    MMNAS_REQUIRE(oc, MMNAS_E_LAUNCH, "chain_bwd: cannot create the encoder stream");
    for (int i = c->n_ops - 1; i >= G; --i)
      if ((rc = run(i, st, cur_dy, &cur_dy))) return rc;
    if ((rc = ev_fork(st, oc->enc, oc->ovl[2]))) return rc;
    const float* enc_dy = nullptr;
    if ((rc = encoder_dy(oc->enc, &enc_dy))) return rc;
    int ie = L.last_x, id = G - 1;
    while (ie >= L.first_x || id >= L.first_y) {
      if (ie >= L.first_x && (rc = run(ie--, oc->enc, enc_dy, &enc_dy))) return rc;
      if (id >= L.first_y && (rc = run(id--, st, cur_dy, &cur_dy))) return rc;
    }
    if ((rc = ev_fork(oc->enc, st, oc->ovl[3]))) return rc;
    if (c->marks)
      for (int i = 0; i < c->n_ops; ++i)
        if (c->marks[i] && hipEventRecord((hipEvent_t)c->marks[i], st) != hipSuccess) {
          set_error("chain_bwd: cannot record the mark event of operator %d", i);
          return MMNAS_E_LAUNCH;
        }
  }
  if (rel_bwd_side && (rc = ev_fork(rel_bwd_side->side, st, rel_bwd_side->ovl[3]))) return rc;
  if (L.first_y < 0 && hipMemcpyAsync(c->dy_in, c->dy_out, ey * sizeof(float), hipMemcpyDeviceToDevice, st) != hipSuccess) return MMNAS_E_LAUNCH;
  if (L.first_x < 0) {
    const float* g0 = c->dx_out;
    if (enc_grad) g0 = enc_grad;
    else if (c->dx_out && L.n_guided) {
      if ((rc = mmnas_drop_add(c->dx_out, dpre, c->dx_in, ex, 0.f, 0, 0, stream))) return rc;
      g0 = nullptr;
    } else if (!c->dx_out) g0 = dpre;
    if (g0 && hipMemcpyAsync(c->dx_in, g0, ex * sizeof(float), hipMemcpyDeviceToDevice, st) != hipSuccess) return MMNAS_E_LAUNCH;
  }
  return MMNAS_OK;
}

extern "C" int mmnas_chain_join(void* main_stream, void* waiting_stream) {
  SideCtx* sc = side_ctx((hipStream_t)main_stream, false);
  if (!sc || !sc->used) return MMNAS_OK;
  hipEvent_t e = sc->ev[MMNAS_CHAIN_MAX_OPS];
  if (hipEventRecord(e, sc->side) != hipSuccess || hipStreamWaitEvent((hipStream_t)waiting_stream, e, 0) != hipSuccess) {
    set_error("chain_join: event record / wait failed");
    return MMNAS_E_LAUNCH;
  }
  return MMNAS_OK;
}

namespace mmnas {

struct HeadSideLayout { float *h, *logit, *probs, *pooled, *dpooled, *dlog, *dh, *dxpool, *g1part; };
static inline int head_rows(const mmnas_head* hd, const mmnas_attflat_side& sd) { return sd.off ? sd.M : hd->B * sd.S; }
struct HeadLayout {
  HeadSideLayout s[2];
  float *xo, *sum, *xy, *dxy, *dsum, *lnws, *g1proj, *dlogT;
  size_t total;
};

static HeadLayout head_layout(const mmnas_head* hd) {
  HeadLayout L;
  Carver c(hd->arena);
  const size_t B = hd->B;
  for (int k = 0; k < 2; ++k) {
    const mmnas_attflat_side& sd = k ? hd->sy : hd->sx;
    const size_t M = sd.off ? (size_t)sd.M : B * sd.S;
    HeadSideLayout& s = L.s[k];
    s.h = c.take(M * hd->MID); s.logit = c.take(M * hd->G); s.probs = c.take(M * hd->G); s.pooled = c.take(B * hd->G * hd->d);
    s.dpooled = c.take(B * hd->G * hd->d); s.dlog = c.take(M * hd->G); s.dh = c.take(M * hd->MID); s.dxpool = c.take(M * hd->d);
    s.g1part = (hd->G == 1 && glimpse1_supported(hd->MID)) ? c.take((size_t)glimpse1_bwd_blocks((long)M, hd->MID) * 3 * hd->MID) : nullptr;
  }
  L.xo = c.take(B * hd->OUT); L.sum = c.take(B * hd->OUT); L.xy = c.take(B * hd->OUT);
  L.dxy = c.take(B * hd->OUT); L.dsum = c.take(B * hd->OUT);
  L.lnws = c.take(mmnas_layernorm_bwd_ws_floats(hd->B, hd->OUT));
  L.g1proj = (hd->ANS == 1 && glimpse1_supported(hd->OUT)) ? c.take((size_t)glimpse1_bwd_blocks((long)B, hd->OUT) * 3 * hd->OUT) : nullptr;
  L.dlogT = (hd->ANS % 4 != 0 && hd->B % 4 == 0 && hd->ANS > 1) ? c.take((size_t)hd->ANS * B) : nullptr;
  L.total = c.off;
  return L;
}

static int head_check(const mmnas_head* hd, const char* who) {
  MMNAS_REQUIRE(hd, MMNAS_E_ARG, "%s: null descriptor", who);
  MMNAS_REQUIRE(hd->B > 0 && hd->d > 0 && hd->MID > 0 && hd->G > 0 && hd->OUT > 0 && hd->ANS > 0 && hd->sx.S > 0 && hd->sy.S > 0,
                MMNAS_E_SHAPE, "%s: B=%d d=%d MID=%d G=%d OUT=%d ANS=%d Sx=%d Sy=%d", who, hd->B, hd->d, hd->MID, hd->G, hd->OUT,
                hd->ANS, hd->sx.S, hd->sy.S);
  MMNAS_REQUIRE(hd->d % 4 == 0 && hd->MID % 4 == 0 && hd->OUT % 4 == 0, MMNAS_E_SHAPE, "%s: d, MID, OUT must be multiples of 4", who);
// ... 80 lines not shown
    return glimpse1_fwd(L.xy, hd->Wp, hd->bp, hd->logits, B, nullptr, nullptr, nullptr, nullptr, 0, OUT, st);
  gemm_init(g, MMNAS_GEMM_NT, hd->ANS, OUT, OUT, OUT, hd->ANS);
  g.g[0].M = B; g.g[0].A[0] = L.xy; g.g[0].B[0] = hd->Wp; g.g[0].bias = hd->bp; g.g[0].C = hd->logits;
  return mmnas_gemm(&g, stream);
}

extern "C" int mmnas_head_bwd(const mmnas_head* hd, void* stream) {
  int rc = head_check(hd, "head_bwd");
  if (rc) return rc;
  MMNAS_REQUIRE(hd->arena && hd->dlogits && hd->ln_a && hd->dln_a && hd->dln_b && hd->Wp && hd->dWp, MMNAS_E_ARG, "head_bwd: null pointer");
  HeadLayout L = head_layout(hd);
  const bool drop = (hd->flags & MMNAS_F_TRAIN) && hd->drop_p > 0.f;
  const float gate_scale = drop ? 1.0f / (1.0f - hd->drop_p) : 1.0f;
  const int B = hd->B, d = hd->d, MID = hd->MID, G = hd->G, OUT = hd->OUT, ANS = hd->ANS;
  hipStream_t st = (hipStream_t)stream;
  mmnas_gemm_desc g, w;
  if (L.g1proj && head_glimpse1_on()) {
    AuxReduce pr;
    if ((rc = glimpse1_bwd(hd->dlogits, L.xy, hd->Wp, 1.0f, 0, L.dxy, nullptr, hd->dWp, L.g1proj, B, OUT, st, &pr))) return rc;
    if ((rc = launch_aux_reduce(pr, st))) return rc;
  } else if (L.dlogT && head_projT_on()) {
    if ((rc = transpose2d(hd->dlogits, L.dlogT, B, ANS, st))) return rc;
    gemm_init(g, MMNAS_GEMM_TN, OUT, ANS, B, OUT, OUT);
    g.g[0].M = B; g.g[0].A[0] = L.dlogT; g.g[0].B[0] = hd->Wp; g.g[0].C = L.dxy;
    if ((rc = mmnas_gemm(&g, stream))) return rc;
    gemm_init(w, MMNAS_GEMM_NN, OUT, B, B, OUT, OUT);
    w.g[0].M = ANS; w.g[0].A[0] = L.dlogT; w.g[0].B[0] = L.xy; w.g[0].C = hd->dWp; w.accumulate = 1;
    if ((rc = mmnas_gemm(&w, stream))) return rc;
  } else {
    gemm_init(w, MMNAS_GEMM_TN, OUT, B, ANS, OUT, OUT);
    w.g[0].M = ANS; w.g[0].A[0] = hd->dlogits; w.g[0].B[0] = L.xy; w.g[0].C = hd->dWp; w.accumulate = 1;
    gemm_init(g, MMNAS_GEMM_NN, OUT, ANS, ANS, OUT, OUT);
    g.g[0].M = B; g.g[0].A[0] = hd->dlogits; g.g[0].B[0] = hd->Wp; g.g[0].C = L.dxy;
    if ((rc = mmnas_gemm_pair(&g, &w, stream))) return rc;
  }
  if (hd->dbp && (rc = mmnas_colsum(hd->dlogits, hd->dbp, B, ANS, ANS, stream))) return rc;
  AuxReduce lnred;
  lnred.part = nullptr;
  if ((rc = layernorm_bwd_deferred(L.sum, hd->ln_a, L.dxy, L.dsum, hd->dln_a, hd->dln_b, nullptr, nullptr, L.lnws, 0.f, 0, 0, B, OUT,
                                   hd->eps, st, &lnred)))
    return rc;
  SideCtx* oc = head_overlap_on() ? side_ctx(st, true) : nullptr;
  if (oc && (rc = ev_fork(st, oc->enc, oc->ovl[2]))) return rc;
  for (int k = 1; k >= 0; --k) {
    const mmnas_attflat_side& sd = k ? hd->sy : hd->sx;
    const HeadSideLayout& s = L.s[k];
    MMNAS_REQUIRE(sd.x && sd.dx && sd.dW1 && sd.dW2 && sd.dWm, MMNAS_E_ARG, "head_bwd: side %d null pointer", k);
    hipStream_t st = (oc && k == 0) ? oc->enc : (hipStream_t)stream;
    void* const stream = (void*)st;
    const int M = head_rows(hd, sd);
    gemm_init(w, MMNAS_GEMM_TN, G * d, B, OUT, G * d, G * d);
    w.g[0].M = OUT; w.g[0].A[0] = L.dsum; w.g[0].B[0] = s.pooled; w.g[0].C = sd.dWm; w.accumulate = 1;
    gemm_init(g, MMNAS_GEMM_NN, G * d, OUT, OUT, G * d, G * d);
    g.g[0].M = B; g.g[0].A[0] = L.dsum; g.g[0].B[0] = sd.Wm; g.g[0].C = s.dpooled;
    if ((rc = gemm_pair_aux(&g, &w, k ? &lnred : nullptr, st))) return rc;
    if (sd.dbm && (rc = mmnas_colsum(L.dsum, sd.dbm, B, OUT, OUT, stream))) return rc;
    if ((rc = sd.off ? attflat_pool_bwd_packed(s.probs, sd.x, s.dpooled, s.dlog, s.dxpool, B, sd.S, d, G, sd.off, st)
                     : mmnas_attflat_pool_bwd(s.probs, sd.x, sd.mask, s.dpooled, s.dlog, s.dxpool, B, sd.S, d, G, stream))) return rc;
    AuxReduce g1red;
    g1red.part = nullptr;
    if (G == 1 && glimpse1_supported(MID) && head_glimpse1_on()) {
      if ((rc = glimpse1_bwd(s.dlog, s.h, sd.W2, gate_scale, 1, s.dh, sd.db1, sd.dW2, s.g1part, M, MID, st, &g1red))) return rc;
      if (sd.db2 && (rc = mmnas_colsum(s.dlog, sd.db2, M, G, G, stream))) return rc;
    } else {
    gemm_init(w, MMNAS_GEMM_TN, MID, M, G, MID, MID);
    w.g[0].M = G; w.g[0].A[0] = s.dlog; w.g[0].B[0] = s.h; w.g[0].C = sd.dW2; w.accumulate = 1;
    gemm_init(g, MMNAS_GEMM_NN, MID, G, G, MID, MID);
    g.g[0].M = M; g.g[0].A[0] = s.dlog; g.g[0].B[0] = sd.W2; g.g[0].C = s.dh;
    g.g[0].gate = s.h; g.ldgate = MID; g.gate_scale = gate_scale;
    g.g[0].colsum = sd.db1;
    if ((rc = mmnas_gemm_pair(&g, &w, stream))) return rc;
    if (sd.db2 && (rc = mmnas_colsum(s.dlog, sd.db2, M, G, G, stream))) return rc;
    }
    gemm_init(w, MMNAS_GEMM_TN, d, M, MID, d, d);
    w.g[0].M = MID; w.g[0].A[0] = s.dh; w.g[0].B[0] = sd.x; w.g[0].C = sd.dW1; w.accumulate = 1;
    gemm_init(g, MMNAS_GEMM_NN, d, MID, MID, d, d);
    g.g[0].M = M; g.g[0].A[0] = s.dh; g.g[0].B[0] = sd.W1; g.g[0].C = sd.dx;
    g.g[0].residual = s.dxpool; g.ldres = d;
    if ((rc = gemm_pair_aux(&g, &w, g1red.part ? &g1red : nullptr, st))) return rc;
  }
  if (oc && (rc = ev_fork(oc->enc, st, oc->ovl[3]))) return rc;
  return MMNAS_OK;
}
```

mmnas_amd/csrc/rowops.hip:

```cpp
#include "common.h"

namespace mmnas {

template <int NV>
__global__ void __launch_bounds__(256) ln_fwd_kernel(const float* __restrict__ x, const float* __restrict__ a,
                                                     const float* __restrict__ b, float* __restrict__ y,
                                                     int M, int d, float eps) {
  const int lane = threadIdx.x & 63;
  const int row = blockIdx.x * 4 + (threadIdx.x >> 6);
  if (row >= M) return;
  const float* xr = x + (size_t)row * d;
  float4 v[NV];
  float s = 0.f;
#pragma unroll
  for (int i = 0; i < NV; ++i) {
    const int c = (lane + 64 * i) * 4;
    v[i] = (c < d) ? *reinterpret_cast<const float4*>(xr + c) : make_float4(0.f, 0.f, 0.f, 0.f);
    s += (v[i].x + v[i].y) + (v[i].z + v[i].w);
  }
  const float mean = wave_sum(s) / (float)d;
  float ss = 0.f;
#pragma unroll
  for (int i = 0; i < NV; ++i) {
    const int c = (lane + 64 * i) * 4;
// ... 85 lines not shown
    const float k2 = sgc / ((float)(d - 1) * sd * sden * sden);
#pragma unroll
    for (int i = 0; i < NV; ++i) {
      const int c = (lane + 64 * i) * 4;
      if (c < d) {
        float4 o;
        o.x = (g[i].x * av[i].x - mg) * inv - v[i].x * k2;
        o.y = (g[i].y * av[i].y - mg) * inv - v[i].y * k2;
        o.z = (g[i].z * av[i].z - mg) * inv - v[i].z * k2;
        o.w = (g[i].w * av[i].w - mg) * inv - v[i].w * k2;
        *reinterpret_cast<float4*>(dx + (size_t)row * d + c) = o;
        acc_a[i].x += g[i].x * v[i].x * inv; acc_a[i].y += g[i].y * v[i].y * inv;
        acc_a[i].z += g[i].z * v[i].z * inv; acc_a[i].w += g[i].w * v[i].w * inv;
        acc_b[i].x += g[i].x; acc_b[i].y += g[i].y; acc_b[i].z += g[i].z; acc_b[i].w += g[i].w;
        if (ddrop) {
          if (drop.thresh) {
            const uint32_t base = (uint32_t)row * (uint32_t)d + (uint32_t)c;
            o.x *= drop_mult(drop, base); o.y *= drop_mult(drop, base + 1);
            o.z *= drop_mult(drop, base + 2); o.w *= drop_mult(drop, base + 3);
          }
          *reinterpret_cast<float4*>(ddrop + (size_t)row * d + c) = o;
          acc_c[i].x += o.x; acc_c[i].y += o.y; acc_c[i].z += o.z; acc_c[i].w += o.w;
        }
      }
    }
  }
  __shared__ __attribute__((aligned(16))) float red[3][4][64 * 4];
#pragma unroll
  for (int i = 0; i < NV; ++i) {
    const int c = (lane + 64 * i) * 4;
    __syncthreads();
    *reinterpret_cast<float4*>(&red[0][wave][lane * 4]) = acc_a[i];
    *reinterpret_cast<float4*>(&red[1][wave][lane * 4]) = acc_b[i];
    *reinterpret_cast<float4*>(&red[2][wave][lane * 4]) = acc_c[i];
    __syncthreads();
    if (wave < 3 && c < d) {
      const f32x4 p0 = *reinterpret_cast<const f32x4*>(&red[wave][0][lane * 4]);
      const f32x4 p1 = *reinterpret_cast<const f32x4*>(&red[wave][1][lane * 4]);
      const f32x4 p2 = *reinterpret_cast<const f32x4*>(&red[wave][2][lane * 4]);
      const f32x4 p3 = *reinterpret_cast<const f32x4*>(&red[wave][3][lane * 4]);
      const f32x4 s4 = (p0 + p1) + (p2 + p3);
      if (part) {
        *reinterpret_cast<f32x4*>(part + ((size_t)blockIdx.x * 3 + wave) * d + c) = s4;
      } else {
        float* out = wave == 0 ? da : (wave == 1 ? db : dcol);
        if (out) {
          atomicAdd(out + c, s4.x); atomicAdd(out + c + 1, s4.y); atomicAdd(out + c + 2, s4.z); atomicAdd(out + c + 3, s4.w);
        }
      }
    }
  }
}

__global__ void __launch_bounds__(1024) ln_bwd_reduce_kernel(const float* __restrict__ part, int nblocks, int d,
                                                             float* __restrict__ da, float* __restrict__ db,
                                                             float* __restrict__ dcol) {
  const int w = blockIdx.y;
  float* out = w == 0 ? da : (w == 1 ? db : dcol);
  if (!out) return;
  const int cl = threadIdx.x & 15, g = threadIdx.x >> 4;
  const int c = blockIdx.x * 16 + cl;
  float s0 = 0.f, s1 = 0.f, s2 = 0.f, s3 = 0.f;
  if (c < d) {
    int b = g;
    for (; b + 192 < nblocks; b += 256) {
      s0 += part[((size_t)b * 3 + w) * d + c];
      s1 += part[((size_t)(b + 64) * 3 + w) * d + c];
      s2 += part[((size_t)(b + 128) * 3 + w) * d + c];
      s3 += part[((size_t)(b + 192) * 3 + w) * d + c];
    }
    for (; b < nblocks; b += 64) s0 += part[((size_t)b * 3 + w) * d + c];
  }
  __shared__ float red[64][17];
  red[g][cl] = (s0 + s1) + (s2 + s3);
  __syncthreads();
  if (g == 0 && c < d) {
    float t = 0.f;
#pragma unroll 8
    for (int i = 0; i < 64; ++i) t += red[i][cl];
    out[c] += t;
  }
}

__global__ void __launch_bounds__(256) colsum_kernel(const float* __restrict__ x, float* __restrict__ out,
                                                     int M, int N, int ldx, int rows_per_block) {
  const int cl = threadIdx.x & 63, g = threadIdx.x >> 6;
  const int col = blockIdx.x * 64 + cl;
  const int r0 = blockIdx.y * rows_per_block;
  const int r1 = min(M, r0 + rows_per_block);
  float s[8];
#pragma unroll
  for (int u = 0; u < 8; ++u) s[u] = 0.f;
  if (col < N) {
    int r = r0 + g;
    for (; r + 28 < r1; r += 32) {
#pragma unroll
      for (int u = 0; u < 8; ++u) s[u] += x[(size_t)(r + 4 * u) * ldx + col];
    }
    for (; r < r1; r += 4) s[0] += x[(size_t)r * ldx + col];
  }
  __shared__ float red[4][64];
  red[g][cl] = ((s[0] + s[1]) + (s[2] + s[3])) + ((s[4] + s[5]) + (s[6] + s[7]));
  __syncthreads();
  if (g == 0 && col < N) atomicAdd(out + col, (red[0][cl] + red[1][cl]) + (red[2][cl] + red[3][cl]));
}

__device__ __forceinline__ float act_fwd(int kind, float x) {
  switch (kind) {
    case 0: return x * 0.f;
    case 1: return fmaxf(x, 0.f);
    case 2: return x > 0.f ? x : 0.01f * x;
    default: {
      const float u = 0.7978845608028654f * (x + 0.044715f * x * x * x);
      return 0.5f * x * (1.f + tanhf(u));
    }
  }
}
__device__ __forceinline__ float act_bwd(int kind, float x) {
  switch (kind) {
    case 0: return 0.f;
    case 1: return x > 0.f ? 1.f : 0.f;
    case 2: return x > 0.f ? 1.f : 0.01f;
    default: {
      const float u = 0.7978845608028654f * (x + 0.044715f * x * x * x);
      const float t = tanhf(u);
      return 0.5f * (1.f + t) + 0.5f * x * (1.f - t * t) * 0.7978845608028654f * (1.f + 3.f * 0.044715f * x * x);
    }
  }
}

__global__ void eltwise_fwd_kernel(int kind, const float* __restrict__ x, float* __restrict__ y, size_t n) {
  for (size_t i = (size_t)blockIdx.x * blockDim.x + threadIdx.x; i < n; i += (size_t)gridDim.x * blockDim.x)
    y[i] = act_fwd(kind, x[i]);
}
__global__ void eltwise_bwd_kernel(int kind, const float* __restrict__ x, const float* __restrict__ dy,
                                   float* __restrict__ dx, size_t n) {
  for (size_t i = (size_t)blockIdx.x * blockDim.x + threadIdx.x; i < n; i += (size_t)gridDim.x * blockDim.x)
    dx[i] = dy[i] * act_bwd(kind, x[i]);
}
__global__ void drop_add_kernel(const float* __restrict__ x, const float* __restrict__ res, float* __restrict__ y,
                                size_t n, DropCfg drop) {
  for (size_t i = (size_t)blockIdx.x * blockDim.x + threadIdx.x; i < n; i += (size_t)gridDim.x * blockDim.x) {
    float v = x[i];
    if (drop.thresh) v *= drop_mult(drop, (uint32_t)i);
    y[i] = res ? res[i] + v : v;
  }
}

struct AddManyK { const float* src[ADD_MANY_MAX]; int n; };
__global__ void add_many_kernel(const AddManyK p, float* __restrict__ y, size_t count4) {
  for (size_t i = (size_t)blockIdx.x * blockDim.x + threadIdx.x; i < count4; i += (size_t)gridDim.x * blockDim.x) {
    float4 acc = reinterpret_cast<const float4*>(p.src[0])[i];
    for (int j = 1; j < p.n; ++j) {
      const float4 v = reinterpret_cast<const float4*>(p.src[j])[i];
      acc.x += v.x; acc.y += v.y; acc.z += v.z; acc.w += v.w;
    }
    reinterpret_cast<float4*>(y)[i] = acc;
  }
}

__global__ void glu_fwd_kernel(const float* __restrict__ h, float* __restrict__ y, int M, int C, int relu,
                               DropCfg drop) {
  const size_t n = (size_t)M * C;
  for (size_t i = (size_t)blockIdx.x * blockDim.x + threadIdx.x; i < n; i += (size_t)gridDim.x * blockDim.x) {
    const size_t m = i / C, c = i - m * C;
    const float a = h[m * 2 * C + c], b = h[m * 2 * C + C + c];
    float v = a / (1.f + expf(-b));
    if (relu) v = fmaxf(v, 0.f);
    if (drop.thresh) v *= drop_mult(drop, (uint32_t)i);
    y[i] = v;
  }
}
__global__ void glu_bwd_kernel(const float* __restrict__ h, const float* __restrict__ dy, float* __restrict__ dh,
                               int M, int C, int relu, DropCfg drop) {
  const size_t n = (size_t)M * C;
  for (size_t i = (size_t)blockIdx.x * blockDim.x + threadIdx.x; i < n; i += (size_t)gridDim.x * blockDim.x) {
    const size_t m = i / C, c = i - m * C;
    const float a = h[m * 2 * C + c], b = h[m * 2 * C + C + c];
    const float sg = 1.f / (1.f + expf(-b));
    float g = dy[i];
    if (drop.thresh) g *= drop_mult(drop, (uint32_t)i);
    if (relu && !(a * sg > 0.f)) g = 0.f;
    dh[m * 2 * C + c] = g * sg;
    dh[m * 2 * C + C + c] = g * a * sg * (1.f - sg);
  }
}

static inline int blocks_for(size_t n) { size_t b = (n + 255) / 256; return (int)(b < 2048 ? (b ? b : 1) : 2048); }

}

using namespace mmnas;

extern "C" int mmnas_layernorm_fwd(const float* x, const float* a, const float* b, float* y, int M, int d,
                                   float eps, void* stream) {
  MMNAS_REQUIRE(x && a && b && y, MMNAS_E_ARG, "layernorm_fwd: null pointer");
  MMNAS_REQUIRE(M > 0 && d >= 4 && d % 4 == 0 && d <= 2048, MMNAS_E_SHAPE,
                "layernorm_fwd: M=%d d=%d (need d %% 4 == 0, 4 <= d <= 2048)", M, d);
  hipStream_t st = (hipStream_t)stream;
  dim3 grid(cdiv(M, 4)), block(256);
  const int nv = cdiv(d, 256);
  ProfScope ps(MMNAS_K_ROWOPS, 8.0 * M * d, 8.0 * M * d, st);
  if (nv <= 1) MMNAS_LAUNCH(ln_fwd_kernel<1>, grid, block, 0, st, x, a, b, y, M, d, eps);
  else if (nv <= 2) MMNAS_LAUNCH(ln_fwd_kernel<2>, grid, block, 0, st, x, a, b, y, M, d, eps);
  else if (nv <= 4) MMNAS_LAUNCH(ln_fwd_kernel<4>, grid, block, 0, st, x, a, b, y, M, d, eps);
  else MMNAS_LAUNCH(ln_fwd_kernel<8>, grid, block, 0, st, x, a, b, y, M, d, eps);
  return check_launch("layernorm_fwd");
}

static int ln_bwd_blocks(int M) {
  int nb = cdiv(M, 4);
  return nb > 512 ? 512 : nb;
}

extern "C" size_t mmnas_layernorm_bwd_ws_floats(int M, int d) { return (size_t)ln_bwd_blocks(M) * 3 * d; }

namespace mmnas {
int layernorm_bwd_deferred(const float* x, const float* a, const float* dy, float* dx, float* da, float* db, float* ddrop,
                           float* dcol, float* ws, float drop_p, uint64_t seed, uint32_t site, int M, int d, float eps,
                           hipStream_t st, AuxReduce* aux) {
  MMNAS_REQUIRE(x && a && dy && dx, MMNAS_E_ARG, "layernorm_bwd: null pointer");
  MMNAS_REQUIRE(M > 0 && d >= 4 && d % 4 == 0 && d <= 2048, MMNAS_E_SHAPE,
                "layernorm_bwd: M=%d d=%d (need d %% 4 == 0, 4 <= d <= 2048)", M, d);
  MMNAS_REQUIRE(dcol == nullptr || ddrop != nullptr, MMNAS_E_ARG, "layernorm_bwd: dcol needs ddrop");
  const int nb = ln_bwd_blocks(M);
  dim3 grid(nb), block(256);
  const DropCfg dc = make_drop(drop_p, seed, site);
  const int nv = cdiv(d, 256);
  ProfScope ps(MMNAS_K_ROWOPS, 16.0 * M * d, 4.0 * M * d * (ddrop ? 4.0 : 3.0), st);
#define LNB(NV) MMNAS_LAUNCH(ln_bwd_kernel<NV>, grid, block, 0, st, x, a, dy, dx, da, db, ddrop, dcol, ws, dc, M, d, eps)
  if (nv <= 1) LNB(1); else if (nv <= 2) LNB(2); else if (nv <= 4) LNB(4); else LNB(8);
#undef LNB
  aux->part = ws; aux->nrows = nb; aux->d = d;
  aux->out[0] = da; aux->out[1] = db; aux->out[2] = dcol;
  if (!ws || (!da && !db && !dcol)) aux->part = nullptr;
  return check_launch("layernorm_bwd");
}

int launch_aux_reduce(const AuxReduce& a, hipStream_t st) {
  if (!a.part) return MMNAS_OK;
  ProfScope ps(MMNAS_K_ROWOPS, 0.0, 4.0 * a.nrows * 3.0 * a.d, st);
  MMNAS_LAUNCH(ln_bwd_reduce_kernel, dim3(cdiv(a.d, 16), 3), dim3(1024), 0, st, a.part, a.nrows, a.d, a.out[0], a.out[1], a.out[2]);
  return check_launch("layernorm_bwd_reduce");
}
}

extern "C" int mmnas_layernorm_bwd(const float* x, const float* a, const float* dy, float* dx, float* da,
                                   float* db, float* ddrop, float* dcol, float* ws, float drop_p, uint64_t seed,
                                   uint32_t site, int M, int d, float eps, void* stream) {
  AuxReduce aux;
  const int rc = layernorm_bwd_deferred(x, a, dy, dx, da, db, ddrop, dcol, ws, drop_p, seed, site, M, d, eps, (hipStream_t)stream, &aux);
  if (rc) return rc;
  return launch_aux_reduce(aux, (hipStream_t)stream);
}

extern "C" int mmnas_colsum(const float* x, float* out, int M, int N, int ldx, void* stream) {
  MMNAS_REQUIRE(x && out && M > 0 && N > 0 && ldx >= N, MMNAS_E_ARG, "colsum: bad arguments");
  int splits = cdiv(M, 64);
  const int colblocks = cdiv(N, 64);
  const int want = cdiv(1024, colblocks);
  if (splits > want) splits = want;
  if (splits < 1) splits = 1;
  const int rpb = cdiv(M, splits);
  MMNAS_LAUNCH(colsum_kernel, dim3(colblocks, cdiv(M, rpb)), dim3(256), 0, (hipStream_t)stream, x, out, M,
                     N, ldx, rpb);
  return check_launch("colsum");
}

extern "C" int mmnas_eltwise_fwd(int kind, const float* x, float* y, size_t n, void* stream) {
  MMNAS_REQUIRE(kind >= 0 && kind <= 3 && x && y, MMNAS_E_ARG, "eltwise_fwd: bad arguments");
  if (n == 0) return MMNAS_OK;
  MMNAS_LAUNCH(eltwise_fwd_kernel, dim3(blocks_for(n)), dim3(256), 0, (hipStream_t)stream, kind, x, y, n);
  return check_launch("eltwise_fwd");
}
extern "C" int mmnas_eltwise_bwd(int kind, const float* x, const float* dy, float* dx, size_t n, void* stream) {
  MMNAS_REQUIRE(kind >= 0 && kind <= 3 && x && dy && dx, MMNAS_E_ARG, "eltwise_bwd: bad arguments");
  if (n == 0) return MMNAS_OK;
  MMNAS_LAUNCH(eltwise_bwd_kernel, dim3(blocks_for(n)), dim3(256), 0, (hipStream_t)stream, kind, x, dy, dx, n);
  return check_launch("eltwise_bwd");
}
extern "C" int mmnas_drop_add(const float* x, const float* res, float* y, size_t n, float drop_p, uint64_t seed,
                              uint32_t site, void* stream) {
  MMNAS_REQUIRE(x && y && n < (1ull << 32), MMNAS_E_ARG, "drop_add: bad arguments");
  if (n == 0) return MMNAS_OK;
  MMNAS_LAUNCH(drop_add_kernel, dim3(blocks_for(n)), dim3(256), 0, (hipStream_t)stream, x, res, y, n,
                     make_drop(drop_p, seed, site));
  return check_launch("drop_add");
}
namespace mmnas {
int add_many(const float* const* srcs, int n, float* y, size_t count, hipStream_t st) {
  MMNAS_REQUIRE(srcs && y && n >= 1 && n <= ADD_MANY_MAX && count % 4 == 0, MMNAS_E_ARG, "add_many: %d sources, %zu elements", n, count);
  AddManyK k;
  k.n = n;
  for (int j = 0; j < n; ++j) { MMNAS_REQUIRE(srcs[j], MMNAS_E_ARG, "add_many: null source %d", j); k.src[j] = srcs[j]; }
  if (count == 0) return MMNAS_OK;
  ProfScope ps(MMNAS_K_ROWOPS, 0.0, 4.0 * (double)count * (n + 1), st);
  MMNAS_LAUNCH(add_many_kernel, dim3(blocks_for(count / 4)), dim3(256), 0, st, k, y, count / 4);
  return check_launch("add_many");
}
}

extern "C" int mmnas_glu_fwd(const float* h, float* y, int M, int C, int relu, float drop_p, uint64_t seed,
                             uint32_t site, void* stream) {
  MMNAS_REQUIRE(h && y && M > 0 && C > 0, MMNAS_E_ARG, "glu_fwd: bad arguments");
  MMNAS_LAUNCH(glu_fwd_kernel, dim3(blocks_for((size_t)M * C)), dim3(256), 0, (hipStream_t)stream, h, y, M, C,
                     relu, make_drop(drop_p, seed, site));
  return check_launch("glu_fwd");
}
extern "C" int mmnas_glu_bwd(const float* h, const float* dy, float* dh, int M, int C, int relu, float drop_p,
                             uint64_t seed, uint32_t site, void* stream) {
  MMNAS_REQUIRE(h && dy && dh && M > 0 && C > 0, MMNAS_E_ARG, "glu_bwd: bad arguments");
  MMNAS_LAUNCH(glu_bwd_kernel, dim3(blocks_for((size_t)M * C)), dim3(256), 0, (hipStream_t)stream, h, dy, dh, M,
                     C, relu, make_drop(drop_p, seed, site));
  return check_launch("glu_bwd");
}
```

mmnas_amd/ops.py:

```python
import ctypes as C
import os
import threading

import torch

from . import _lib as L

_seed_lock = threading.Lock()
_seed_state = {'base': None, 'counter': 0}


def manual_seed(seed):
    with _seed_lock:
        _seed_state['base'] = int(seed) & 0xFFFFFFFFFFFFFFFF
        _seed_state['counter'] = 0


def next_seed():
    with _seed_lock:
        if _seed_state['base'] is None:
            _seed_state['base'] = int(torch.initial_seed()) & 0xFFFFFFFFFFFFFFFF
        _seed_state['counter'] += 1
        x = (_seed_state['base'] * 0x9E3779B97F4A7C15 + _seed_state['counter'] * 0xD1B54A32D192ED03)
        return x & 0xFFFFFFFFFFFFFFFF


_plan_cache = {}
_sinks_on = [True]


def runtime_config():
    return {
        'lib_path': L.LIB_PATH,
        'lib_loaded': L._lib is not None,
        'abi_version': L.lib().mmnas_abi_version() if os.path.exists(L.LIB_PATH) else None,
        'hip_force_dev_kernarg': os.environ.get('HIP_FORCE_DEV_KERNARG'),
        'hip_force_dev_kernarg_source': L.KERNARG_SOURCE,
        'hip_initialised': torch.cuda.is_initialized(),
        'torch': torch.__version__, 'hip': getattr(torch.version, 'hip', None),
        'env': {k: v for k, v in sorted(os.environ.items()) if k.startswith(('MMNAS_', 'HIP_', 'NCCL_', 'RCCL_', 'HSA_'))},
    }


class no_sinks:

    def __enter__(self):
        self._old = _sinks_on[0]
        _sinks_on[0] = False

    def __exit__(self, *a):
        _sinks_on[0] = self._old



def _grad_bufs(params, dev):
    bufs, rets, sinks, fresh = [], [], [], []
    for t in params:
        if t is None:
            bufs.append(None); rets.append(None)
            continue
        s = getattr(t, '_mmnas_sink', None)
        if s is not None and t.grad is s.view and _sinks_on[0]:
            bufs.append(s.view); rets.append(None); sinks.append(s)
        else:
            bufs.append(t); rets.append(t); fresh.append(len(bufs) - 1)
    if fresh:
        sizes = [bufs[i].numel() for i in fresh]
        flat = torch.zeros(sum(sizes), dtype=torch.float32, device=dev)
        for i, part in zip(fresh, torch.split(flat, sizes)):
            g = part.view(bufs[i].shape)
            bufs[i] = g
            rets[i] = g
    return bufs, rets, sinks


def _bytes(n, dev):
    return torch.empty(max(int(n), 256), dtype=torch.uint8, device=dev)


def _f32c(t):
    if t.dtype != torch.float32:
        raise L.MMNasHipError('mmnas_amd operators compute in float32; got %s' % t.dtype)
    return t.contiguous()


def _mask_u8(mask, B, Sk):
    if mask is None:
        return None
    m = mask.reshape(B, Sk)
    if m.dtype == torch.bool:
        m = m.contiguous().view(torch.uint8)
    elif m.dtype != torch.uint8:
        m = (m != 0).to(torch.uint8)
    return m.contiguous()


class AttentionOp(torch.autograd.Function):

    @staticmethod
    def forward(ctx, xq, xkv, mask, rel, Wq, Wk, Wv, Wm, Wr, br, ln_a, ln_b, Wy, by, dh, norm, residual, drop_p,
                training, seed, eps):
        lib = L.lib()
        self_att = xkv is None or xkv is xq
        xq = _f32c(xq)
        xkv = xq if self_att else _f32c(xkv)
        B, Sq, d = xq.shape
        Sk = xkv.shape[1]
        di = Wq.shape[0]
        H = di // dh
        dev = xq.device
        flags = (L.F_NORM if norm else 0) | (L.F_RESIDUAL if residual else 0)
        if self_att:
            flags |= L.F_SELF
        m8 = _mask_u8(mask, B, Sk)
        if m8 is not None:
            flags |= L.F_MASK
        lazy = rel is not None and Wy is not None
        if rel is not None:
            rel = _f32c(rel)
            want = (B, Sq, Sk, Wy.shape[1] if lazy else Wr.shape[1])
            if tuple(rel.shape) != want:
# ... 320 lines not shown
        if ctx.has_bias:
            L.check(L.lib().mmnas_colsum(L.fptr(dy), L.fptr(db), M, N, N, L.stream()))
        for sk in sinks:
            sk.done()
        return dx, rets[0], rets[1], None


class EmbeddingFn(torch.autograd.Function):

    @staticmethod
    def forward(ctx, idx, weight):
        ctx.weight = weight
        ctx.save_for_backward(idx)
        ctx.rows_key = None
        s = getattr(weight, '_mmnas_sink', None)
        rows = getattr(s.owner, 'row_exchange', None) if s is not None and s.owner is not None else None
        if rows is not None and rows.active and rows.i == s.index and weight.grad is s.view and _sinks_on[0] and ctx.needs_input_grad[1]:
            ctx.rows_key = rows.gather_indices(idx)
        return torch.nn.functional.embedding(idx, weight)

    @staticmethod
    def backward(ctx, dy):
        idx, = ctx.saved_tensors
        w = ctx.weight
        dy = _f32c(dy)
        idx = idx.contiguous()
        (dW,), rets, sinks = _grad_bufs([w], dy.device)
        rows = getattr(sinks[0].owner, 'row_exchange', None) if sinks and sinks[0].owner is not None else None
        if rows is not None and rows.active and rows.i == sinks[0].index:
            rows.exchange(idx, dy, ctx.rows_key)
        else:
            L.check(L.lib().mmnas_embedding_bwd(L.ptr(idx), L.fptr(dy), L.fptr(dW), idx.numel(), w.shape[1], w.shape[0], L.stream()))
        for sk in sinks:
            sk.done()
        return None, rets[0]


def embedding(idx, mod):
    if (idx.is_cuda and idx.dtype == torch.int64 and mod.weight.dtype == torch.float32 and mod.padding_idx is None
            and mod.max_norm is None and not mod.sparse and not mod.scale_grad_by_freq):
        return EmbeddingFn.apply(idx, mod.weight)
    return mod(idx)


class LstmFn(torch.autograd.Function):

    @staticmethod
    def forward(ctx, x, w_ih, w_hh, b_ih, b_hh):
        lib = L.lib()
        ctx.params = (w_ih, w_hh, b_ih, b_hh)
        x, Wih, Whh = _f32c(x), _f32c(w_ih), _f32c(w_hh)
        B, T, E = x.shape
        H = Whh.shape[1]
        dev = x.device
        xp = torch.empty(B, T, 4 * H, dtype=torch.float32, device=dev)
        gemm(L.GEMM_NT, [dict(M=B * T, A=[x], B=[Wih], C=xp, bias=_f32c(b_ih))], 4 * H, E, E, E, 4 * H)
        st = torch.empty(3, B, T, H, dtype=torch.float32, device=dev)
        Gall = torch.empty(B, T, 4 * H, dtype=torch.float32, device=dev)
        L.check(lib.mmnas_lstm_seq_fwd(L.fptr(xp), L.fptr(_f32c(b_hh)), L.fptr(Whh), L.fptr(st[0]), L.fptr(st[1]), L.fptr(Gall),
                                       L.fptr(st[2]), T, B, H, L.stream()))
        ctx.save_for_backward(x, Wih, Whh, st, Gall)
        ctx.dims = (B, T, E, H)
        return st[2]

    @staticmethod
    def backward(ctx, dout):
        lib = L.lib()
        x, Wih, Whh, st, Gall = ctx.saved_tensors
        B, T, E, H = ctx.dims
        dev = dout.device
        dout = _f32c(dout)
        DG = torch.empty(B, T, 4 * H, dtype=torch.float32, device=dev)
        L.check(lib.mmnas_lstm_seq_bwd(L.fptr(dout), L.fptr(Whh), L.fptr(st[1]), L.fptr(Gall), L.fptr(DG), T, B, H, L.stream()))
        (dWih, dWhh, dbih, dbhh), rets, sinks = _grad_bufs(ctx.params, dev)
        M = B * T
        wg_ih = gemm_desc(L.GEMM_TN, [dict(M=4 * H, A=[DG], B=[x], C=dWih)], E, M, 4 * H, E, E, accumulate=True)
        dx = None
        if ctx.needs_input_grad[0]:
            dx = torch.empty_like(x)
            gemm_pair(gemm_desc(L.GEMM_NN, [dict(M=M, A=[DG], B=[Wih], C=dx)], E, 4 * H, 4 * H, E, E), wg_ih)
        else:
            L.check(lib.mmnas_gemm(C.byref(wg_ih), L.stream()))
        gemm(L.GEMM_TN, [dict(M=4 * H, A=[DG], B=[st[0]], C=dWhh)], H, M, 4 * H, H, H, accumulate=True)
        L.check(lib.mmnas_colsum(L.fptr(DG), L.fptr(dbih), M, 4 * H, 4 * H, L.stream()))
        L.check(lib.mmnas_colsum(L.fptr(DG), L.fptr(dbhh), M, 4 * H, 4 * H, L.stream()))
        for sk in sinks:
            sk.done()
        return dx, rets[0], rets[1], rets[2], rets[3]


def lstm(x, mod):
    return LstmFn.apply(x, mod.weight_ih_l0, mod.weight_hh_l0, mod.bias_ih_l0, mod.bias_hh_l0)


def lstm_enabled():
    import os
    return os.environ.get('MMNAS_LSTM', '1') != '0'


def lstm_supported(x, mod):
    return (x.is_cuda and x.dtype == torch.float32 and x.dim() == 3 and mod.num_layers == 1 and not mod.bidirectional
            and mod.batch_first and mod.bias and mod.proj_size == 0 and mod.input_size % 4 == 0
            and bool(L.lib().mmnas_lstm_seq_supported(mod.hidden_size, x.shape[0])))


def linear(x, W, b=None, relu=False):
    return LinearFn.apply(x, W, b, relu)


class LayerNormFn(torch.autograd.Function):

    @staticmethod
    def forward(ctx, x, a, b, eps):
        x, a, b = _f32c(x), _f32c(a), _f32c(b)
        d = x.shape[-1]
        M = x.numel() // d
        y = torch.empty_like(x)
        L.check(L.lib().mmnas_layernorm_fwd(L.fptr(x), L.fptr(a), L.fptr(b), L.fptr(y), M, d, eps, L.stream()))
        ctx.save_for_backward(x, a)
        ctx.eps = eps
        return y

    @staticmethod
    def backward(ctx, dy):
        x, a = ctx.saved_tensors
        dy = _f32c(dy)
        d = x.shape[-1]
        M = x.numel() // d
        dx = torch.empty_like(x)
        dab = torch.zeros(2, d, dtype=torch.float32, device=x.device)
        ws = torch.empty(L.lib().mmnas_layernorm_bwd_ws_floats(M, d), dtype=torch.float32, device=x.device)
        L.check(L.lib().mmnas_layernorm_bwd(L.fptr(x), L.fptr(a), L.fptr(dy), L.fptr(dx), L.fptr(dab[0]),
                                            L.fptr(dab[1]), None, None, L.fptr(ws), 0.0, 0, 0, M, d, ctx.eps,
                                            L.stream()))
        return dx, dab[0], dab[1], None


def layer_norm(x, a, b, eps=1e-6):
    return LayerNormFn.apply(x, a, b, eps)


class EltwiseFn(torch.autograd.Function):

    @staticmethod
    def forward(ctx, x, kind):
        x = _f32c(x)
        y = torch.empty_like(x)
        L.check(L.lib().mmnas_eltwise_fwd(kind, L.fptr(x), L.fptr(y), x.numel(), L.stream()))
        ctx.save_for_backward(x)
        ctx.kind = kind
        return y

    @staticmethod
    def backward(ctx, dy):
        (x,) = ctx.saved_tensors
        dy = _f32c(dy)
        dx = torch.empty_like(x)
        L.check(L.lib().mmnas_eltwise_bwd(ctx.kind, L.fptr(x), L.fptr(dy), L.fptr(dx), x.numel(), L.stream()))
        return dx, None


def eltwise(x, kind):
    return EltwiseFn.apply(x, kind)


class GluFn(torch.autograd.Function):

    @staticmethod
# ... 858 lines not shown
```

Before: 224.5 steps/s.

## Add deferred wgrad GEMMs riding in tri-product launches; fuse LSTM bias colsums

Adds an opt-in queue that defers weight-gradient GEMMs during chain backward and packs each one into a later dgrad/wgrad pair launch through a new three-product kernel, or pairs them at flush points. The aim is to fill idle workgroup slots within the resident budget and cut launch count. The LSTM backward now computes both bias gradients with one colsum kernel that writes two outputs. The deferral is off unless an environment variable enables it, and it adds planning logic and a larger kernel-argument block.

```diff
diff --git a/include/mmnas_hip.h b/include/mmnas_hip.h
--- a/include/mmnas_hip.h
+++ b/include/mmnas_hip.h
@@ -96,6 +96,7 @@
 size_t mmnas_layernorm_bwd_ws_floats(int M, int d);
 
 int mmnas_colsum(const float* x, float* out, int M, int N, int ldx, void* stream);
+int mmnas_colsum2(const float* x, float* out, float* out2, int M, int N, int ldx, void* stream);
 
 int mmnas_eltwise_fwd(int kind, const float* x, float* y, size_t n, void* stream);
 int mmnas_eltwise_bwd(int kind, const float* x, const float* dy, float* dx, size_t n, void* stream);
@@ -243,6 +244,11 @@
 
 int mmnas_set_small_ops(int on);
 int mmnas_set_small_bwd(int on);
+
+int mmnas_set_defer_wgrad(int on);
+int mmnas_get_defer_wgrad(void);
+int mmnas_defer_wgrad_plan(int n, const int* kind, const int* ngroups, const int* nwg, const int* event_after, int enabled, int budget,
+                           int* launch_of, int* launch_kind, int* launch_nwg, int* launch_groups, int* event_launches, int* n_launches);
 int mmnas_set_small_ffn(int on);
 int mmnas_att_op_plan(const mmnas_att_op* op, mmnas_plan* plan);
 int mmnas_att_op_fwd(const mmnas_att_op* op, void* stream);
diff --git a/mmnas_amd/_lib.py b/mmnas_amd/_lib.py
--- a/mmnas_amd/_lib.py
+++ b/mmnas_amd/_lib.py
@@ -150,6 +150,9 @@
     'mmnas_lstm_seq_supported': (_i, [_i, _i]),
     'mmnas_set_small_ops': (_i, [_i]),
     'mmnas_set_small_bwd': (_i, [_i]),
+    'mmnas_set_defer_wgrad': (_i, [_i]),
+    'mmnas_get_defer_wgrad': (_i, []),
+    'mmnas_defer_wgrad_plan': (_i, [_i] + [C.POINTER(C.c_int)] * 4 + [_i, _i] + [C.POINTER(C.c_int)] * 6),
     'mmnas_set_small_ffn': (_i, [_i]),
     'mmnas_set_chain_overlap': (_i, [_i]),
     'mmnas_lstm_seq_fwd': (_i, [_fp] * 7 + [_i, _i, _i, _fp]),
@@ -159,6 +162,7 @@
     'mmnas_layernorm_bwd': (_i, [_fp, _fp, _fp, _fp, _fp, _fp, _fp, _fp, _fp, _f, _u64, _u32, _i, _i, _f, _fp]),
     'mmnas_layernorm_bwd_ws_floats': (_sz, [_i, _i]),
     'mmnas_colsum': (_i, [_fp, _fp, _i, _i, _i, _fp]),
+    'mmnas_colsum2': (_i, [_fp, _fp, _fp, _i, _i, _i, _fp]),
     'mmnas_eltwise_fwd': (_i, [_i, _fp, _fp, _sz, _fp]),
     'mmnas_eltwise_bwd': (_i, [_i, _fp, _fp, _fp, _sz, _fp]),
     'mmnas_drop_add': (_i, [_fp, _fp, _fp, _sz, _f, _u64, _u32, _fp]),
diff --git a/mmnas_amd/csrc/common.h b/mmnas_amd/csrc/common.h
--- a/mmnas_amd/csrc/common.h
+++ b/mmnas_amd/csrc/common.h
@@ -74,6 +74,10 @@
 int launch_aux_reduce(const AuxReduce& a, hipStream_t st);
 int gemm_pair_aux(const mmnas_gemm_desc* dgrad, const mmnas_gemm_desc* wgrad, const AuxReduce* aux, hipStream_t st);
 int gemm_wgrad_aux(const mmnas_gemm_desc* wgrad, const AuxReduce* aux, hipStream_t st);
+int gemm_resident_wgs();
+int gemm_pair_nwg(const mmnas_gemm_desc* dgrad, const mmnas_gemm_desc* wgrad, const AuxReduce* aux, hipStream_t st, int* nwg, bool* tri);
+int gemm_tri_aux(const mmnas_gemm_desc* dgrad, const mmnas_gemm_desc* wgrad, const AuxReduce* aux, const mmnas_gemm_desc* ride,
+                 const AuxReduce* ride_aux, hipStream_t st);
 int layernorm_bwd_deferred(const float* x, const float* a, const float* dy, float* dx, float* da, float* db, float* ddrop,
                            float* dcol, float* ws, float drop_p, uint64_t seed, uint32_t site, int M, int d, float eps,
                            hipStream_t st, AuxReduce* aux);
diff --git a/mmnas_amd/csrc/gemm.hip b/mmnas_amd/csrc/gemm.hip
--- a/mmnas_amd/csrc/gemm.hip
+++ b/mmnas_amd/csrc/gemm.hip
@@ -955,6 +955,31 @@
     gemm_body<BM, BN, false, false, true, NS, 0, PF, false, LEAN1>(q1, bid - nwg0p, (int)gridDim.x - naux8 - nwg0p, (int)sizeof(GemmK), As, Bs, As1, Bs1, s_old);
   }
 }
+
+template <int LEAN0>
+__global__ void __launch_bounds__(256, MMNAS_OCC_NS) gemm_tri_kernel(const GemmK q0, const GemmK q1, const GemmK q2, const int nwg0,
+                                                                     const int nwg0p, const int nwg1, const int nwg1p,
+                                                                     const AuxReduceK aux0, const AuxReduceK aux1, const int naux8_0,
+                                                                     const int naux8) {
+  __shared__ __attribute__((aligned(16))) float As[GemmShape<64, 64, 3>::A_SZ], As1[GemmShape<64, 64, 3>::A_SZ];
+  __shared__ __attribute__((aligned(16))) float Bs[GemmShape<64, 64, 3>::B_SZ], Bs1[GemmShape<64, 64, 3>::B_SZ];
+  __shared__ int s_old;
+  int bid = blockIdx.x;
+  if (bid < naux8) {
+    if (bid < naux8_0) { if (bid < aux0.njobs) aux_reduce_body(aux0, bid, As); }
+    else if (bid - naux8_0 < aux1.njobs) aux_reduce_body(aux1, bid - naux8_0, As);
+    return;
+  }
+  bid -= naux8;
+  if (bid < nwg0p) {
+    if (bid < nwg0) gemm_body<64, 64, true, false, true, 3, 0, 2, false, LEAN0>(q0, bid, nwg0, 0, As, Bs, As1, Bs1, s_old);
+  } else if (bid < nwg0p + nwg1p) {
+    if (bid - nwg0p < nwg1) gemm_body<64, 64, false, false, true, 3, 0, 2, false, 1>(q1, bid - nwg0p, nwg1, (int)sizeof(GemmK), As, Bs, As1, Bs1, s_old);
+  } else {
+    gemm_body<64, 64, false, false, true, 3, 0, 2, false, 1>(q2, bid - nwg0p - nwg1p, (int)gridDim.x - naux8 - nwg0p - nwg1p, 2 * (int)sizeof(GemmK), As, Bs, As1, Bs1, s_old);
+  }
+}
+static_assert(3 * sizeof(GemmK) + 2 * sizeof(AuxReduceK) + 6 * sizeof(int) <= 4096, "gemm_tri_kernel: the arguments must fit one 4 KB kernel-argument block");
 
 static int env_int(const char* name, int dflt) {
   const char* e = getenv(name);
@@ -1364,6 +1389,67 @@
 }
 }
 
+namespace mmnas {
+static void aux_to_k(const AuxReduce* aux, AuxReduceK& ak) {
+  memset(&ak, 0, sizeof(ak));
+  if (!aux || !aux->part) return;
+  ak.part = aux->part; ak.nrows = aux->nrows; ak.d = aux->d;
+  for (int i = 0; i < 3; ++i) ak.out[i] = aux->out[i];
+  ak.ncb = cdiv(aux->d, 16);
+  ak.njobs = 3 * ak.ncb;
+}
+
+int gemm_resident_wgs() {
+  static const int n = [] {
+    int dev = 0, cus = 0;
+    if (hipGetDevice(&dev) != hipSuccess || hipDeviceGetAttribute(&cus, hipDeviceAttributeMultiprocessorCount, dev) != hipSuccess || cus <= 0) cus = 256;
+    return cus * MMNAS_OCC_NS;
+  }();
+  return n;
+}
+
+int gemm_pair_nwg(const mmnas_gemm_desc* dgrad, const mmnas_gemm_desc* wgrad, const AuxReduce* aux, hipStream_t st, int* nwg, bool* tri) {
+  GemmPlan p0, p1;
+  int rc;
+  *nwg = 0; *tri = false;
+  if (dgrad && (rc = plan_gemm(dgrad, st, p0))) return rc;
+  if ((rc = plan_gemm(wgrad, st, p1))) return rc;
+  const int naux8 = (aux && aux->part) ? (3 * cdiv(aux->d, 16) + 7) / 8 * 8 : 0;
+  *nwg = naux8 + (dgrad ? (p0.nwg + 7) / 8 * 8 : 0) + (p1.nwg + 7) / 8 * 8;
+  *tri = g_tune.pair && g_tune.pair != 3 && g_tune.split == 3 && g_tune.pf == 2 && p1.fast && !p1.big && !p1.wide && p1.layout == MMNAS_GEMM_TN &&
+         p1.lean == 1 && (!dgrad || (p0.fast && !p0.big && !p0.wide && p0.layout == MMNAS_GEMM_NN && p0.lean >= 1 && p0.lean <= 3));
+  return MMNAS_OK;
+}
+
+int gemm_tri_aux(const mmnas_gemm_desc* dgrad, const mmnas_gemm_desc* wgrad, const AuxReduce* aux, const mmnas_gemm_desc* ride,
+                 const AuxReduce* ride_aux, hipStream_t st) {
+  GemmPlan p0, p1, p2;
+  int rc;
+  if (dgrad && (rc = plan_gemm(dgrad, st, p0))) return rc;
+  if ((rc = plan_gemm(wgrad, st, p1))) return rc;
+  if ((rc = plan_gemm(ride, st, p2))) return rc;
+  MMNAS_REQUIRE(g_tune.split == 3 && g_tune.pf == 2 && p1.lean == 1 && p2.lean == 1 && p1.layout == MMNAS_GEMM_TN && p2.layout == MMNAS_GEMM_TN &&
+                    (!dgrad || (p0.layout == MMNAS_GEMM_NN && p0.lean >= 1 && p0.lean <= 3)),
+                MMNAS_E_ARG, "gemm_tri_aux: a product outside the lean split-operand kernels");
+  AuxReduceK a0, a1;
+  aux_to_k(aux, a0);
+  aux_to_k(ride_aux, a1);
+  const int naux8_0 = (a0.njobs + 7) / 8 * 8, naux8 = naux8_0 + (a1.njobs + 7) / 8 * 8;
+  const int nwg0 = dgrad ? p0.nwg : 0, nwg0p = (nwg0 + 7) / 8 * 8, nwg1p = (p1.nwg + 7) / 8 * 8;
+  char tag[96] = "";
+  if (prof_enabled()) snprintf(tag, sizeof(tag), "TRI %.30s | %.26s | %.26s", dgrad ? p0.tag : "-", p1.tag, p2.tag);
+  ProfScope ps(MMNAS_K_GEMM, (dgrad ? p0.flops : 0.0) + p1.flops + p2.flops, (dgrad ? p0.bytes : 0.0) + p1.bytes + p2.bytes, st, tag);
+  const dim3 grid(naux8 + nwg0p + nwg1p + p2.nwg), block(256);
+  const GemmK& k0 = dgrad ? p0.k : p1.k;
+  switch (dgrad ? p0.lean : 1) {
+    case 3: MMNAS_LAUNCH((gemm_tri_kernel<3>), grid, block, 0, st, k0, p1.k, p2.k, nwg0, nwg0p, p1.nwg, nwg1p, a0, a1, naux8_0, naux8); break;
+    case 2: MMNAS_LAUNCH((gemm_tri_kernel<2>), grid, block, 0, st, k0, p1.k, p2.k, nwg0, nwg0p, p1.nwg, nwg1p, a0, a1, naux8_0, naux8); break;
+    default: MMNAS_LAUNCH((gemm_tri_kernel<1>), grid, block, 0, st, k0, p1.k, p2.k, nwg0, nwg0p, p1.nwg, nwg1p, a0, a1, naux8_0, naux8); break;
+  }
+  return check_launch("gemm_tri");
+}
+}
+
 extern "C" int mmnas_gemm_pair(const mmnas_gemm_desc* dgrad, const mmnas_gemm_desc* wgrad, void* stream) {
   return gemm_pair_aux(dgrad, wgrad, nullptr, (hipStream_t)stream);
 }
diff --git a/mmnas_amd/csrc/ops.hip b/mmnas_amd/csrc/ops.hip
--- a/mmnas_amd/csrc/ops.hip
+++ b/mmnas_amd/csrc/ops.hip
@@ -227,8 +227,71 @@
   }
 };
 
+static int g_defer_wgrad = -1;
+static bool defer_wgrad_on() {
+  if (g_defer_wgrad < 0) { const char* e = getenv("MMNAS_DEFER_WGRAD"); g_defer_wgrad = (e && e[0] ? atoi(e) : 0) ? 1 : 0; }
+  return g_defer_wgrad != 0;
+}
+
+struct DeferPlanner {
+  struct Item { int id, ngroups, nwg; };
+  int budget = 0;
+  std::vector<Item> q;
+  void defer(int id, int ngroups, int nwg) { q.push_back({id, ngroups, nwg}); }
+  int ride(int nwg) {
+    if (q.empty() || nwg + q.front().nwg > budget) return -1;
+    const int id = q.front().id;
+    q.erase(q.begin());
+    return id;
+  }
+  bool flush_next(int* a, int* b) {
+    if (q.empty()) return false;
+    *a = q.front().id; *b = -1;
+    const int n0 = q.front().nwg;
+    q.erase(q.begin());
+    if (!q.empty() && n0 + q.front().nwg <= budget) { *b = q.front().id; q.erase(q.begin()); }
+    return true;
+  }
+};
+
+struct DeferQueue {
+  struct Entry { mmnas_gemm_desc w; AuxReduce red; int nwg; };
+  std::vector<Entry> items;
+  DeferPlanner plan;
+  hipStream_t st = nullptr;
+  int defer(const mmnas_gemm_desc& w, const AuxReduce& red) {
+    int nwg = 0; bool tri = false;
+    int rc = gemm_pair_nwg(nullptr, &w, &red, st, &nwg, &tri);
+    if (rc) return rc;
+    if (!tri) return gemm_wgrad_aux(&w, &red, st);
+    items.push_back({w, red, nwg});
+    plan.defer((int)items.size() - 1, w.ngroups, nwg);
+    return MMNAS_OK;
+  }
+  int pair(const mmnas_gemm_desc* g, const mmnas_gemm_desc* w, const AuxReduce* aux) {
+    if (!plan.q.empty()) {
+      int nwg = 0; bool tri = false;
+      int rc = gemm_pair_nwg(g, w, aux, st, &nwg, &tri);
+      if (rc) return rc;
+      const int id = tri ? plan.ride(nwg) : -1;
+      if (id >= 0) return gemm_tri_aux(g, w, aux, &items[id].w, &items[id].red, st);
+    }
+    return gemm_pair_aux(g, w, aux, st);
+  }
+  int flush() {
+    int a, b, rc;
+    while (plan.flush_next(&a, &b)) {
+      if (b < 0) rc = gemm_wgrad_aux(&items[a].w, &items[a].red, st);
+      else rc = gemm_tri_aux(nullptr, &items[a].w, &items[a].red, &items[b].w, &items[b].red, st);
+      if (rc) return rc;
+    }
+    items.clear();
+    return MMNAS_OK;
+  }
+};
+
 static int att_bwd_impl(const mmnas_att_op* op, hipStream_t stream, SideQueue* sq, bool acc_kv = false, bool rel_defer = false, bool kv_defer = false,
-                        const AuxReduce* ln_pre = nullptr) {
+                        const AuxReduce* ln_pre = nullptr, DeferQueue* dq = nullptr) {
   const bool side = sq != nullptr && !sq->rel_only;
   const bool side_rel = sq != nullptr;
   int rc = att_check(op, "att_op_bwd");
@@ -259,6 +322,7 @@
     AuxReduce red;
     red.part = norm ? L.lnws : nullptr; red.nrows = op->B; red.d = d;
     red.out[0] = op->dln_a; red.out[1] = op->dln_b; red.out[2] = nullptr;
+    if (dq) return dq->defer(w4, red);
     return gemm_wgrad_aux(&w4, &red, stream);
   }
 
@@ -286,7 +350,7 @@
   wm.g[0].M = d; wm.g[0].A[0] = dt; wm.g[0].B[0] = L.att; wm.g[0].C = op->dWm;
   wm.accumulate = 1;
   if (side) { if ((rc = mmnas_gemm(&g, stream))) return rc; }
-  else if ((rc = gemm_pair_aux(&g, &wm, &lnred, (hipStream_t)stream))) return rc;
+  else if ((rc = dq ? dq->pair(&g, &wm, &lnred) : gemm_pair_aux(&g, &wm, &lnred, (hipStream_t)stream))) return rc;
 
   mmnas_mha_desc m;
   memset(&m, 0, sizeof(m));
@@ -315,7 +379,7 @@
     if (fl & MMNAS_F_RESIDUAL) { g.g[0].residual = dz; g.ldres = d; }
     if (side) {
       if ((rc = mmnas_gemm(&g, stream))) return rc;
-    } else if ((rc = mmnas_gemm_pair(&g, &w, stream))) return rc;
+    } else if ((rc = dq ? dq->pair(&g, &w, nullptr) : mmnas_gemm_pair(&g, &w, stream))) return rc;
   } else {
     gemm_init(w, MMNAS_GEMM_TN, d, Mq, di, d, d);
     w.g[0].M = di; w.g[0].A[0] = L.dQ; w.g[0].B[0] = op->xq; w.g[0].C = op->dWq;
@@ -325,7 +389,7 @@
     if (fl & MMNAS_F_RESIDUAL) { g.g[0].residual = dz; g.ldres = d; }
     if (side) {
       if ((rc = mmnas_gemm(&g, stream))) return rc;
-    } else if ((rc = mmnas_gemm_pair(&g, &w, stream))) return rc;
+    } else if ((rc = dq ? dq->pair(&g, &w, nullptr) : mmnas_gemm_pair(&g, &w, stream))) return rc;
     if (kv_defer) goto params;
     gemm_init(w2, MMNAS_GEMM_TN, d, Mk, di, d, d);
     w2.ngroups = 2;
@@ -340,7 +404,7 @@
     if (acc_kv) g.accumulate = 1;
     if (side) {
       if ((rc = mmnas_gemm(&g, stream))) return rc;
-    } else if ((rc = mmnas_gemm_pair(&g, &w2, stream))) return rc;
+    } else if ((rc = dq ? dq->pair(&g, &w2, nullptr) : mmnas_gemm_pair(&g, &w2, stream))) return rc;
   }
 
 params:
@@ -478,7 +542,7 @@
 }
 
 namespace mmnas {
-static int mlp_bwd_impl(const mmnas_mlp_op* op, hipStream_t stream, SideQueue* sq, const AuxReduce* ln_pre = nullptr) {
+static int mlp_bwd_impl(const mmnas_mlp_op* op, hipStream_t stream, SideQueue* sq, const AuxReduce* ln_pre = nullptr, DeferQueue* dq = nullptr) {
   const bool side = sq != nullptr && !sq->rel_only;
   int rc = mlp_check(op, "mlp_op_bwd");
   if (rc) return rc;
@@ -537,7 +601,8 @@
     }
     if (side) {
       if ((rc = mmnas_gemm(&g, stream))) return rc;
-    } else if ((rc = gemm_pair_aux(&g, &w, i == nl - 1 ? &lnred : nullptr, (hipStream_t)stream))) return rc;
+    } else if ((rc = dq ? dq->pair(&g, &w, i == nl - 1 ? &lnred : nullptr)
+                        : gemm_pair_aux(&g, &w, i == nl - 1 ? &lnred : nullptr, (hipStream_t)stream))) return rc;
     if (i > 0) dpre = g.g[0].C;
   }
   if (side) {
@@ -1115,6 +1180,9 @@
   RelGroups RG;
   chain_rel_groups(c, L, true, RG);
   SideCtx* rel_bwd_side = nullptr;
+  DeferQueue dqs;
+  dqs.st = st; dqs.plan.budget = gemm_resident_wgs();
+  DeferQueue* const dq = defer_wgrad_on() ? &dqs : nullptr;
   for (int k = nn - 1; k >= 0; --k) {
     const int i0 = starts[k], i1 = starts[k + 1];
     const bool oy = c->ops[i0].on_y;
@@ -1190,16 +1258,17 @@
     }
     if (o.kind == MMNAS_CHAIN_ATT) {
       const bool self = a.flags & MMNAS_F_SELF;
-      if ((rc = att_bwd_impl(&a, st, nullptr, !self, RG.hoisted[act_op], GS.hoisted[act_op], lnb.dz ? &lnpre : nullptr))) return rc;
+      if ((rc = att_bwd_impl(&a, st, nullptr, !self, RG.hoisted[act_op], GS.hoisted[act_op], lnb.dz ? &lnpre : nullptr, dq))) return rc;
       if (GS.n && act_op == Gm) {
         float* g0 = (float*)(base + L.encdy);
         if ((rc = chain_guided_kv_bwd(c, L, GS, x_final, c->dx_out, GS.n < L.n_guided ? dpre : nullptr, g0, st))) return rc;
         enc_grad = g0;
       }
     } else {
-      if ((rc = mlp_bwd_impl(&m, st, nullptr, lnb.dz ? &lnpre : nullptr))) return rc;
+      if ((rc = mlp_bwd_impl(&m, st, nullptr, lnb.dz ? &lnpre : nullptr, dq))) return rc;
     }
     cur_dy = dx;
+    if (dq && c->marks && c->marks[act_op] && (rc = dq->flush())) return rc;
     hipStream_t mark_stream = st;
     if (i0 == L.first_y && !RG.groups[1].empty()) {
       SideCtx* rsc = (rel_overlap_on() && L.last_x >= 0) ? side_ctx(st, true) : nullptr;
@@ -1219,6 +1288,7 @@
       return MMNAS_E_LAUNCH;
     }
   }
+  if (dq && (rc = dq->flush())) return rc;
   if (rel_bwd_side && (rc = ev_fork(rel_bwd_side->side, st, rel_bwd_side->ovl[3]))) return rc;
   if (n_red && (rc = mixed_reduce_many(red_part, red_out, red_nwg, red_n, n_red, st))) return rc;
   if (L.first_y < 0 && hipMemcpyAsync(c->dy_in, c->dy_out, ey * sizeof(float), hipMemcpyDeviceToDevice, st) != hipSuccess) return MMNAS_E_LAUNCH;
@@ -1324,6 +1394,8 @@
   SideQueue q;
   q.rel_only = c->use_side_stream == 2;
   SideQueue* sq = sc ? &q : nullptr;
+  DeferQueue dqs;
+  dqs.st = st; dqs.plan.budget = gemm_resident_wgs();
   static const bool per_op = getenv("MMNAS_SIDE_FLUSH") && !strcmp(getenv("MMNAS_SIDE_FLUSH"), "op");
   char* base = (char*)c->arena;
   const size_t ex = (size_t)c->B * c->Sx * c->d, ey = chain_rows_y(c) * c->d;
@@ -1337,6 +1409,7 @@
   const float* x_final = L.last_x >= 0 ? c->x_out : c->x_in;
   const int G = first_guided(c);
   const bool ovl = chain_overlap_on() && !c->use_side_stream && L.last_x >= 0 && L.first_y >= 0 && G > L.first_y;
+  DeferQueue* const dq = (defer_wgrad_on() && !sq && !ovl) ? &dqs : nullptr;
   RelGroups RG;
   if (!ovl) chain_rel_groups(c, L, true, RG);
   GuidedSet GS;
@@ -1358,7 +1431,7 @@
       a.dy = dyi; a.dxq = dx;
       a.dxkv = self ? nullptr : dpre;
       a.drel = nullptr;
-      if ((r = att_bwd_impl(&a, s, sq, !self, RG.hoisted[i], GS.hoisted[i]))) return r;
+      if ((r = att_bwd_impl(&a, s, sq, !self, RG.hoisted[i], GS.hoisted[i], nullptr, dq))) return r;
       if (GS.n && i == G) {
         float* g0 = (float*)(base + L.encdy);
         if ((r = chain_guided_kv_bwd(c, L, GS, x_final, c->dx_out, GS.n < L.n_guided ? dpre : nullptr, g0, s))) return r;
@@ -1367,9 +1440,10 @@
     } else {
       m.x = input_of(i); m.save = base + L.save[i]; m.ws = base + L.ws[i];
       m.dy = dyi; m.dx = dx;
-      if ((r = mlp_bwd_impl(&m, s, sq))) return r;
+      if ((r = mlp_bwd_impl(&m, s, sq, nullptr, dq))) return r;
     }
     *dxo = dx;
+    if (dq && c->marks && c->marks[i] && (r = dq->flush())) return r;
     hipStream_t mark_stream = s;
     if (i == L.first_y && !RG.groups[1].empty()) {
       SideCtx* rsc = (rel_overlap_on() && L.last_x >= 0 && !sq) ? side_ctx(st, true) : nullptr;
@@ -1410,6 +1484,7 @@
       if (sq && per_op && (rc = q.flush(st, side, sc->ev[i + 1]))) return rc;
     }
     if (sq && (rc = q.flush(st, side, sc->ev[1]))) return rc;
+    if (dq && (rc = dq->flush())) return rc;
   } else {
     SideCtx* oc = side_ctx(st, true);
     MMNAS_REQUIRE(oc, MMNAS_E_LAUNCH, "chain_bwd: cannot create the encoder stream");
@@ -1656,3 +1731,50 @@
   if (oc && (rc = ev_fork(oc->enc, st, oc->ovl[3]))) return rc;
   return MMNAS_OK;
 }
+
+extern "C" int mmnas_set_defer_wgrad(int on) {
+  const int prev = mmnas::defer_wgrad_on() ? 1 : 0;
+  mmnas::g_defer_wgrad = on ? 1 : 0;
+  return prev;
+}
+
+extern "C" int mmnas_get_defer_wgrad(void) { return mmnas::defer_wgrad_on() ? 1 : 0; }
+
+extern "C" int mmnas_defer_wgrad_plan(int n, const int* kind, const int* ngroups, const int* nwg, const int* event_after, int enabled, int budget,
+                                      int* launch_of, int* launch_kind, int* launch_nwg, int* launch_groups, int* event_launches, int* n_launches) {
+  MMNAS_REQUIRE(n >= 0 && (n == 0 || (kind && ngroups && nwg && event_after && launch_of && launch_kind && launch_nwg && launch_groups && event_launches)) &&
+                    n_launches, MMNAS_E_ARG, "defer_wgrad_plan: null pointer");
+  mmnas::DeferPlanner pl;
+  pl.budget = budget > 0 ? budget : mmnas::gemm_resident_wgs();
+  int nl = 0;
+  auto flush = [&]() {
+    int a, b;
+    while (pl.flush_next(&a, &b)) {
+      launch_kind[nl] = 2;
+      launch_nwg[nl] = nwg[a] + (b >= 0 ? nwg[b] : 0);
+      launch_groups[nl] = b >= 0 && ngroups[b] > ngroups[a] ? ngroups[b] : ngroups[a];
+      launch_of[a] = nl;
+      if (b >= 0) launch_of[b] = nl;
+      ++nl;
+    }
+  };
+  for (int i = 0; i < n; ++i) {
+    MMNAS_REQUIRE((kind[i] == 0 || kind[i] == 1) && ngroups[i] >= 1 && ngroups[i] <= MMNAS_GEMM_MAX_GROUPS && nwg[i] >= 1, MMNAS_E_ARG,
+                  "defer_wgrad_plan: product %d: kind %d, %d groups, %d workgroups", i, kind[i], ngroups[i], nwg[i]);
+    if (kind[i] == 1 && enabled) pl.defer(i, ngroups[i], nwg[i]);
+    else {
+      const int r = (kind[i] == 0 && enabled) ? pl.ride(nwg[i]) : -1;
+      launch_kind[nl] = kind[i] == 1 ? 3 : (r >= 0 ? 1 : 0);
+      launch_nwg[nl] = nwg[i] + (r >= 0 ? nwg[r] : 0);
+      launch_groups[nl] = r >= 0 && ngroups[r] > ngroups[i] ? ngroups[r] : ngroups[i];
+      launch_of[i] = nl;
+      if (r >= 0) launch_of[r] = nl;
+      ++nl;
+    }
+    event_launches[i] = -1;
+    if (event_after[i]) { flush(); event_launches[i] = nl; }
+  }
+  flush();
+  *n_launches = nl;
+  return MMNAS_OK;
+}
diff --git a/mmnas_amd/csrc/rowops.hip b/mmnas_amd/csrc/rowops.hip
--- a/mmnas_amd/csrc/rowops.hip
+++ b/mmnas_amd/csrc/rowops.hip
@@ -191,7 +191,7 @@
   }
 }
 
-__global__ void __launch_bounds__(256) colsum_kernel(const float* __restrict__ x, float* __restrict__ out,
+__global__ void __launch_bounds__(256) colsum_kernel(const float* __restrict__ x, float* __restrict__ out, float* __restrict__ out2,
                                                      int M, int N, int ldx, int rows_per_block) {
   const int cl = threadIdx.x & 63, g = threadIdx.x >> 6;
   const int col = blockIdx.x * 64 + cl;
@@ -211,7 +211,11 @@
   __shared__ float red[4][64];
   red[g][cl] = ((s[0] + s[1]) + (s[2] + s[3])) + ((s[4] + s[5]) + (s[6] + s[7]));
   __syncthreads();
-  if (g == 0 && col < N) atomicAdd(out + col, (red[0][cl] + red[1][cl]) + (red[2][cl] + red[3][cl]));
+  if (g == 0 && col < N) {
+    const float t = (red[0][cl] + red[1][cl]) + (red[2][cl] + red[3][cl]);
+    atomicAdd(out + col, t);
+    if (out2) atomicAdd(out2 + col, t);
+  }
 }
 
 __device__ __forceinline__ float act_fwd(int kind, float x) {
@@ -364,14 +368,18 @@
 }
 
 extern "C" int mmnas_colsum(const float* x, float* out, int M, int N, int ldx, void* stream) {
-  MMNAS_REQUIRE(x && out && M > 0 && N > 0 && ldx >= N, MMNAS_E_ARG, "colsum: bad arguments");
+  return mmnas_colsum2(x, out, nullptr, M, N, ldx, stream);
+}
+
+extern "C" int mmnas_colsum2(const float* x, float* out, float* out2, int M, int N, int ldx, void* stream) {
+  MMNAS_REQUIRE(x && out && M > 0 && N > 0 && ldx >= N && out2 != out, MMNAS_E_ARG, "colsum: bad arguments");
   int splits = cdiv(M, 64);
   const int colblocks = cdiv(N, 64);
   const int want = cdiv(1024, colblocks);
   if (splits > want) splits = want;
   if (splits < 1) splits = 1;
   const int rpb = cdiv(M, splits);
-  MMNAS_LAUNCH(colsum_kernel, dim3(colblocks, cdiv(M, rpb)), dim3(256), 0, (hipStream_t)stream, x, out, M,
+  MMNAS_LAUNCH(colsum_kernel, dim3(colblocks, cdiv(M, rpb)), dim3(256), 0, (hipStream_t)stream, x, out, out2, M,
                      N, ldx, rpb);
   return check_launch("colsum");
 }
diff --git a/mmnas_amd/ops.py b/mmnas_amd/ops.py
--- a/mmnas_amd/ops.py
+++ b/mmnas_amd/ops.py
@@ -37,6 +37,7 @@
         'hip_force_dev_kernarg': os.environ.get('HIP_FORCE_DEV_KERNARG'),
         'hip_force_dev_kernarg_source': L.KERNARG_SOURCE,
         'hip_initialised': torch.cuda.is_initialized(),
+        'defer_wgrad': bool(L.lib().mmnas_get_defer_wgrad()) if os.path.exists(L.LIB_PATH) else None,
         'torch': torch.__version__, 'hip': getattr(torch.version, 'hip', None),
         'env': {k: v for k, v in sorted(os.environ.items()) if k.startswith(('MMNAS_', 'HIP_', 'NCCL_', 'RCCL_', 'HSA_'))},
     }
@@ -523,8 +524,7 @@
         else:
             L.check(lib.mmnas_gemm(C.byref(wg_ih), L.stream()))
         gemm(L.GEMM_TN, [dict(M=4 * H, A=[DG], B=[st[0]], C=dWhh)], H, M, 4 * H, H, H, accumulate=True)
-        L.check(lib.mmnas_colsum(L.fptr(DG), L.fptr(dbih), M, 4 * H, 4 * H, L.stream()))
-        L.check(lib.mmnas_colsum(L.fptr(DG), L.fptr(dbhh), M, 4 * H, 4 * H, L.stream()))
+        L.check(lib.mmnas_colsum2(L.fptr(DG), L.fptr(dbih), L.fptr(dbhh), M, 4 * H, 4 * H, L.stream()))
         for sk in sinks:
             sk.done()
         return dx, rets[0], rets[1], rets[2], rets[3]
```

Measured after the change: 225.0 steps/s, median of 6. About the same (+0.2%).
